# cbacary/MoDeGPT

Hardware: AMD Instinct MI355X
Metric: transformer layers compressed/sec (covariance+decomp+rebuild), Llama-3-8B @30% (higher is better)
Workload: dtype f64 from int8 MFMA digit planes, exact route: nine plane pairs + fp64 remainder sums, nothing truncated (error <= 5e-15 per call: fp64 rounding)

## Files before the change

modegpt_amd/csrc/common.hpp:

```cpp
#pragma once
#include <hip/hip_runtime.h>
#include <hip/hip_bf16.h>
#include <hip/hip_fp16.h>
#include <stdint.h>
#include <stdio.h>
#include <string.h>

#include "../../include/modegpt_hip.h"

namespace mdg {

typedef double d4 __attribute__((ext_vector_type(4)));
typedef double d2 __attribute__((ext_vector_type(2)));
typedef unsigned short bf16_t;
typedef unsigned short f16_t;

#ifdef MDG_EXPERIMENT
#define MDG_KNOB(name) (getenv(name) != nullptr)
#else
#define MDG_KNOB(name) false
#endif

void set_error(const char* fmt, ...);
enum { STATUS_NOT_PD = 1, STATUS_NO_CONVERGE = 2 };
int finish_flag(int* dflag, hipStream_t st, int kind, const char* what);

int release_i8_schedules();
int cov_accum_gated(const void* x, int dtype, int64_t n_tokens, int64_t n_feat, int64_t batch, int64_t ld, int relu, double* sigma,
                    int64_t ld_sigma, int64_t sigma_bs, void* ws, size_t ws_bytes, const int* gate, int gate_mask, int gate_want,
                    void* stream);
#define MDG_CHECK_ARG(cond, ...)            \
  do {                                      \
    if (!(cond)) {                          \
      mdg::set_error(__VA_ARGS__);          \
      return MDG_ERR_BAD_ARG;               \
    }                                       \
  } while (0)
#define MDG_HIP(call)                                                        \
  do {                                                                       \
    hipError_t e_ = (call);                                                  \
    if (e_ != hipSuccess) {                                                  \
      mdg::set_error("%s failed: %s (%s:%d)", #call, hipGetErrorString(e_),  \
                     __FILE__, __LINE__);                                    \
      return MDG_ERR_HIP;                                                    \
    }                                                                        \
  } while (0)
#define MDG_LAUNCH_CHECK() MDG_HIP(hipGetLastError())
#define MDG_CLEAR() (void)hipGetLastError()
#define MDG_TRY(call)              \
  do {                             \
    int s_ = (call);               \
    if (s_ != MDG_OK) return s_;   \
  } while (0)

__device__ __forceinline__ double bf16_to_f64(bf16_t b) {
  return (double)__uint_as_float(((unsigned)b) << 16);
}
__device__ __forceinline__ double f16_to_f64(f16_t h) {
  __half_raw r;
  r.x = h;
  return (double)__half2float(__half(r));
}
__device__ __forceinline__ bf16_t f64_to_bf16(double v) {
  float f = (float)v;
  unsigned u = __float_as_uint(f);
  if ((u & 0x7fffffffu) > 0x7f800000u) return (bf16_t)0x7fc0;
  u += 0x7fffu + ((u >> 16) & 1u);
  return (bf16_t)(u >> 16);
}

template <int DT> struct ElemOf;
template <> struct ElemOf<MDG_BF16> { typedef bf16_t type; };
template <> struct ElemOf<MDG_F16> { typedef f16_t type; };
template <> struct ElemOf<MDG_F32> { typedef float type; };
template <> struct ElemOf<MDG_F64> { typedef double type; };

template <int DT> __device__ __forceinline__ double load_f64(const void* p, int64_t i);
template <> __device__ __forceinline__ double load_f64<MDG_BF16>(const void* p, int64_t i) {
  return bf16_to_f64(((const bf16_t*)p)[i]);
}
template <> __device__ __forceinline__ double load_f64<MDG_F16>(const void* p, int64_t i) {
  return f16_to_f64(((const f16_t*)p)[i]);
}
template <> __device__ __forceinline__ double load_f64<MDG_F32>(const void* p, int64_t i) {
  return (double)((const float*)p)[i];
}
template <> __device__ __forceinline__ double load_f64<MDG_F64>(const void* p, int64_t i) {
  return ((const double*)p)[i];
}

static inline size_t dtype_size(int dt) {
  switch (dt) {
    case MDG_BF16: case MDG_F16: return 2;
    case MDG_F32: return 4;
    case MDG_F64: return 8;
  }
  return 0;
}

static inline int64_t ceil_div(int64_t a, int64_t b) { return (a + b - 1) / b; }
static inline size_t align_up(size_t a, size_t b) { return (a + b - 1) / b * b; }

constexpr int TILE = 128;
constexpr int WTILE = 64;
constexpr int BK = 16;
constexpr int PITCH = TILE + 2;
constexpr int PANEL = BK * PITCH;

struct Acc {
  d4 v[4][4];
};

__device__ __forceinline__ void acc_zero(Acc& a) {
#pragma unroll
  for (int i = 0; i < 4; i++)
#pragma unroll
    for (int j = 0; j < 4; j++) a.v[i][j] = (d4){0., 0., 0., 0.};
}

template <int K4_LO, int K4_HI>
__device__ __forceinline__ void mma_steps(const double* __restrict__ As, const double* __restrict__ Bs, int wr,
                                          int wc, int lane, Acc& acc) {
  const int m = lane & 15, kq = lane >> 4;
#pragma unroll
  for (int k4 = K4_LO; k4 < K4_HI; k4++) {
    const double* ap = As + (k4 * 4 + kq) * PITCH + wr * WTILE + 4 * m;
    const double* bp = Bs + (k4 * 4 + kq) * PITCH + wc * WTILE + 4 * m;
    d2 a01 = *(const d2*)ap, a23 = *(const d2*)(ap + 2);
    d2 b01 = *(const d2*)bp, b23 = *(const d2*)(bp + 2);
    double a[4] = {a01.x, a01.y, a23.x, a23.y};
    double b[4] = {b01.x, b01.y, b23.x, b23.y};
#pragma unroll
    for (int sa = 0; sa < 4; sa++)
#pragma unroll
      for (int sb = 0; sb < 4; sb++)
        acc.v[sa][sb] = __builtin_amdgcn_mfma_f64_16x16x4f64(a[sa], b[sb], acc.v[sa][sb], 0, 0, 0);
  }
}

__device__ __forceinline__ void mma_stage(const double* __restrict__ As, const double* __restrict__ Bs, int wr,
                                          int wc, int lane, Acc& acc) {
  mma_steps<0, BK / 4>(As, Bs, wr, wc, lane, acc);
}

__device__ __forceinline__ int acc_row(int wr, int lane, int sa, int reg) {
  return wr * WTILE + 4 * ((lane >> 4) + 4 * reg) + sa;
}
__device__ __forceinline__ int acc_col(int wc, int lane, int sb) { return wc * WTILE + 4 * (lane & 15) + sb; }

__device__ __forceinline__ void tri_decode(int t, int& bi, int& bj) {
  int i = (int)((sqrt(8.0 * (double)t + 1.0) - 1.0) * 0.5);
  while ((i + 1) * (i + 2) / 2 <= t) i++;
  while (i * (i + 1) / 2 > t) i--;
  bi = i;
  bj = t - i * (i + 1) / 2;
}

}
```

modegpt_amd/csrc/cov.hip:

```cpp
#include <stdlib.h>

#include <type_traits>

#include "common.hpp"

namespace mdg {

struct CovArgs {
  const void* x;
  int64_t ld, n_tokens;
  int n_feat, batch, tiles, ntri;
  double* sigma;
  int64_t ld_sigma, sigma_bs;
  int ksplit;
  int64_t tokens_per_split;
  double* partial;
  int vec_ok;
  const int* gate;
  int gate_mask, gate_want;
};

template <int DT> struct Stage {
  typedef typename ElemOf<DT>::type T;
  static constexpr int VEC = 16 / (int)sizeof(T);
  static constexpr int CPR = TILE / VEC;
  static constexpr int CPT = BK * CPR / 256;
  union Chunk {
    uint4 q;
    T e[VEC];
  };
  static constexpr int RG = VEC >= 8 ? 4 : (VEC == 4 ? 2 : 1);
  static constexpr int CG = 8 / RG;
  __device__ static __forceinline__ void chunk_rc(int c, int& row, int& col) {
    const int g = c >> 3, i = c & 7;
    row = (g % (BK / RG)) * RG + (i % RG);
    col = ((g / (BK / RG)) * CG + i / RG) * VEC;
  }
};

template <int DT, bool FAST, bool INB = false>
__device__ __forceinline__ void load_panel(const CovArgs& a, int64_t tok0, int64_t tok_end, int64_t col0,
                                           int col_lim, int tid, typename Stage<DT>::Chunk* regs) {
  typedef Stage<DT> S;
  typedef typename S::T T;
  const T* x = (const T*)a.x;
#pragma unroll
  for (int p = 0; p < S::CPT; p++) {
    int row, col;
    S::chunk_rc(tid + 256 * p, row, col);
    int64_t tok = tok0 + row;
    typename S::Chunk ch;
    ch.q = make_uint4(0, 0, 0, 0);
    if (FAST && INB) {
      ch.q = *(const uint4*)(x + tok * a.ld + col0 + col);
    } else if (FAST) {
      if (tok < tok_end) ch.q = *(const uint4*)(x + tok * a.ld + col0 + col);
    } else if (tok < tok_end) {
      const T* src = x + tok * a.ld + col0 + col;
      if (a.vec_ok && col + S::VEC <= col_lim) {
        ch.q = *(const uint4*)src;
      } else {
#pragma unroll
        for (int e = 0; e < S::VEC; e++)
          if (col + e < col_lim) ch.e[e] = src[e];
      }
    }
    regs[p] = ch;
  }
}

template <int DT, bool RELU>
__device__ __forceinline__ void store_panel(double* panel, int tid, const typename Stage<DT>::Chunk* regs) {
  typedef Stage<DT> S;
#pragma unroll
  for (int p = 0; p < S::CPT; p++) {
    int row, col;
    S::chunk_rc(tid + 256 * p, row, col);
    double* dst = panel + row * PITCH + col;
#pragma unroll
    for (int e = 0; e < S::VEC; e += 2) {
      double v0 = load_f64<DT>(regs[p].e, e), v1 = load_f64<DT>(regs[p].e, e + 1);
      if (RELU) {
        v0 = v0 > 0. ? v0 : 0.;
        v1 = v1 > 0. ? v1 : 0.;
      }
      *(d2*)(dst + e) = (d2){v0, v1};
    }
  }
}

template <int DT, bool RELU>
__device__ __forceinline__ void store_piece(double* panel, int tid, const typename Stage<DT>::Chunk* regs, int piece) {
  typedef Stage<DT> S;
  constexpr int PAIRS = S::CPT * S::VEC / 2;
  constexpr int PER = PAIRS / 4;
#pragma unroll
  for (int u = 0; u < PER; u++) {
    const int w = piece * PER + u;
    const int p = w / (S::VEC / 2), e = (w % (S::VEC / 2)) * 2;
    int row, col;
    S::chunk_rc(tid + 256 * p, row, col);
    double v0 = load_f64<DT>(regs[p].e, e), v1 = load_f64<DT>(regs[p].e, e + 1);
    if (RELU) {
      v0 = v0 > 0. ? v0 : 0.;
      v1 = v1 > 0. ? v1 : 0.;
    }
    *(d2*)(panel + row * PITCH + col + e) = (d2){v0, v1};
  }
}

template <int DT, bool RELU, bool DIAG>
__device__ __forceinline__ void mma_half_with_staging(const double* __restrict__ As, const double* __restrict__ Bs,
                                                      int wr, int wc, int lane, Acc& acc, bool stage_next,
                                                      double* nextA, double* nextB, int tid,
                                                      const typename Stage<DT>::Chunk* ra,
                                                      const typename Stage<DT>::Chunk* rb) {
  const int m = lane & 15, kq = lane >> 4;
  double a[2][4], b[2][4];
#pragma unroll
  for (int h = 0; h < 2; h++) {
    const int k4 = BK / 8 + h;
    const double* ap = As + (k4 * 4 + kq) * PITCH + wr * WTILE + 4 * m;
    const double* bp = Bs + (k4 * 4 + kq) * PITCH + wc * WTILE + 4 * m;
    d2 a01 = *(const d2*)ap, a23 = *(const d2*)(ap + 2);
    d2 b01 = *(const d2*)bp, b23 = *(const d2*)(bp + 2);
    a[h][0] = a01.x; a[h][1] = a01.y; a[h][2] = a23.x; a[h][3] = a23.y;
    b[h][0] = b01.x; b[h][1] = b01.y; b[h][2] = b23.x; b[h][3] = b23.y;
  }
#pragma unroll
  for (int h = 0; h < 2; h++)
#pragma unroll
    for (int sa = 0; sa < 4; sa++) {
#pragma unroll
      for (int sb = 0; sb < 4; sb++)
        acc.v[sa][sb] = __builtin_amdgcn_mfma_f64_16x16x4f64(a[h][sa], b[h][sb], acc.v[sa][sb], 0, 0, 0);
      if (stage_next) {
        const int piece = h * 4 + sa;
        if (piece < 4) store_piece<DT, RELU>(nextA, tid, ra, piece);
        else if (!DIAG) store_piece<DT, RELU>(nextB, tid, rb, piece - 4);
      }
      __builtin_amdgcn_sched_barrier(0);
    }
}

template <int DT, bool RELU, bool FAST, bool DIAG>
__device__ __forceinline__ void cov_tile(const CovArgs& a, double* lds, int b, int bi, int bj, int split, int slot) {
  typedef Stage<DT> S;
  const int tid = threadIdx.x, lane = tid & 63, wave = tid >> 6;
  const int wr = wave >> 1, wc = wave & 1;
  const int64_t tok_begin = (int64_t)split * a.tokens_per_split;
  int64_t tok_end = tok_begin + a.tokens_per_split;
  if (tok_end > a.n_tokens) tok_end = a.n_tokens;
  const int64_t colA = (int64_t)b * a.n_feat + (int64_t)bi * TILE;
  const int64_t colB = (int64_t)b * a.n_feat + (int64_t)bj * TILE;
  const int limA = min(TILE, a.n_feat - bi * TILE), limB = min(TILE, a.n_feat - bj * TILE);

  Acc acc;
  acc_zero(acc);
  typename S::Chunk ra1[S::CPT], rb1[S::CPT], ra2[S::CPT], rb2[S::CPT];
  const int64_t n_stage = tok_end > tok_begin ? (tok_end - tok_begin + BK - 1) / BK : 0;

  if (n_stage > 0) {
    load_panel<DT, FAST>(a, tok_begin, tok_end, colA, limA, tid, ra1);
    if (!DIAG) load_panel<DT, FAST>(a, tok_begin, tok_end, colB, limB, tid, rb1);
    store_panel<DT, RELU>(lds, tid, ra1);
    if (!DIAG) store_panel<DT, RELU>(lds + 2 * PANEL, tid, rb1);
    if (n_stage > 1) {
      load_panel<DT, FAST>(a, tok_begin + BK, tok_end, colA, limA, tid, ra1);
      if (!DIAG) load_panel<DT, FAST>(a, tok_begin + BK, tok_end, colB, limB, tid, rb1);
    }
  }
  __syncthreads();
  auto stage = [&](int64_t s, auto cur_c, auto steady_c, typename S::Chunk* st_a, typename S::Chunk* st_b,
                   typename S::Chunk* ld_a, typename S::Chunk* ld_b) {
    constexpr int CUR = decltype(cur_c)::value;
    constexpr bool STEADY = decltype(steady_c)::value;
    if (STEADY || s + 2 < n_stage) {
      const int64_t tk = tok_begin + (s + 2) * BK;
      load_panel<DT, FAST, STEADY>(a, tk, tok_end, colA, limA, tid, ld_a);
      if (!DIAG) load_panel<DT, FAST, STEADY>(a, tk, tok_end, colB, limB, tid, ld_b);
    }
    const double* As = lds + CUR * PANEL;
    const double* Bs = DIAG ? As : lds + (2 + CUR) * PANEL;
    mma_steps<0, BK / 8>(As, Bs, wr, wc, lane, acc);
    mma_half_with_staging<DT, RELU, DIAG>(As, Bs, wr, wc, lane, acc, STEADY || s + 1 < n_stage, lds + (CUR ^ 1) * PANEL,
                                          lds + (2 + (CUR ^ 1)) * PANEL, tid, st_a, st_b);
    __syncthreads();
  };
  using I0 = std::integral_constant<int, 0>;
  using I1 = std::integral_constant<int, 1>;
  int64_t s = 0;
  const int64_t n_full = (tok_end - tok_begin) / BK;
  for (; s + 3 < n_full; s += 2) {
    stage(s, I0{}, std::true_type{}, ra1, rb1, ra2, rb2);
    stage(s + 1, I1{}, std::true_type{}, ra2, rb2, ra1, rb1);
  }
  for (; s + 1 < n_stage; s += 2) {
    stage(s, I0{}, std::false_type{}, ra1, rb1, ra2, rb2);
    stage(s + 1, I1{}, std::false_type{}, ra2, rb2, ra1, rb1);
  }
  if (s < n_stage) stage(s, I0{}, std::false_type{}, ra1, rb1, ra2, rb2);

  if (a.ksplit == 1) {
    double* sg = a.sigma + (int64_t)b * a.sigma_bs;
#pragma unroll
    for (int sa = 0; sa < 4; sa++)
#pragma unroll
      for (int reg = 0; reg < 4; reg++) {
        int r = acc_row(wr, lane, sa, reg);
        int64_t gr = (int64_t)bi * TILE + r;
        if (gr >= a.n_feat) continue;
        int c0 = acc_col(wc, lane, 0);
        int64_t gc0 = (int64_t)bj * TILE + c0;
        double* row = sg + gr * a.ld_sigma + gc0;
#pragma unroll
        for (int sb = 0; sb < 4; sb++)
          if (gc0 + sb < a.n_feat) row[sb] += acc.v[sa][sb][reg];
      }
  } else {
    double* pt = a.partial + ((int64_t)split * (a.batch * a.ntri) + slot) * (TILE * TILE);
#pragma unroll
    for (int sa = 0; sa < 4; sa++)
#pragma unroll
      for (int reg = 0; reg < 4; reg++) {
        int r = acc_row(wr, lane, sa, reg);
        int c0 = acc_col(wc, lane, 0);
        d4 v = {acc.v[sa][0][reg], acc.v[sa][1][reg], acc.v[sa][2][reg], acc.v[sa][3][reg]};
        *(d4*)(pt + r * TILE + c0) = v;
      }
  }
}

template <int DT, bool RELU, bool FAST>
__global__ __launch_bounds__(256, 2) void cov_accum_kernel(CovArgs a) {
  __shared__ double lds[4 * PANEL];
  if (a.gate && (*a.gate & a.gate_mask) != a.gate_want) return;
  const int b = blockIdx.x / a.ntri, t = blockIdx.x % a.ntri;
  int bi, bj;
  tri_decode(t, bi, bj);
  if (bi == bj) cov_tile<DT, RELU, FAST, true>(a, lds, b, bi, bj, blockIdx.y, blockIdx.x);
  else cov_tile<DT, RELU, FAST, false>(a, lds, b, bi, bj, blockIdx.y, blockIdx.x);
}

constexpr int MULTI_MAX = 4;
struct CovMulti {
  int n;
  int unit_start[MULTI_MAX + 1];
  CovArgs p[MULTI_MAX];
};

template <int DT>
__global__ __launch_bounds__(256, 2) void cov_accum_multi_kernel(CovMulti m) {
  __shared__ double lds[4 * PANEL];
  int u = blockIdx.x, pi = 0;
  while (pi + 1 < m.n && u >= m.unit_start[pi + 1]) pi++;
  u -= m.unit_start[pi];
  const CovArgs& a = m.p[pi];
  const int tiles = a.batch * a.ntri;
  const int split = u / tiles, slot = u % tiles;
  const int b = slot / a.ntri, t = slot % a.ntri;
  int bi, bj;
  tri_decode(t, bi, bj);
  if (bi == bj) cov_tile<DT, false, true, true>(a, lds, b, bi, bj, split, slot);
  else cov_tile<DT, false, true, false>(a, lds, b, bi, bj, split, slot);
}

__global__ __launch_bounds__(256) void cov_reduce_kernel(CovArgs a) {
  if (a.gate && (*a.gate & a.gate_mask) != a.gate_want) return;
  const int b = blockIdx.x / a.ntri, t = blockIdx.x % a.ntri;
  int bi, bj;
  tri_decode(t, bi, bj);
  double* sg = a.sigma + (int64_t)b * a.sigma_bs;
  const int64_t tile_stride = (int64_t)gridDim.x * (TILE * TILE);
  const double* pt = a.partial + (int64_t)blockIdx.x * (TILE * TILE);
  const int e = blockIdx.y * 256 + threadIdx.x;
  const int r = e / TILE, c = e % TILE;
  const int64_t gr = (int64_t)bi * TILE + r, gc = (int64_t)bj * TILE + c;
  if (gr >= a.n_feat || gc >= a.n_feat) return;
  double s = 0.;
  for (int k = 0; k < a.ksplit; k++) s += pt[k * tile_stride + e];
  sg[gr * a.ld_sigma + gc] += s;
}

__global__ __launch_bounds__(256) void cov_finalize_kernel(double* sigma, int n, int64_t ld, int64_t bs, int tiles,
                                                           int ntri, double scale) {
  __shared__ double tl[32][33];
  const int b = blockIdx.x / ntri, t = blockIdx.x % ntri;
  int ti, tj;
  tri_decode(t, ti, tj);
  double* sg = sigma + (int64_t)b * bs;
  const int tx = threadIdx.x & 31, ty = threadIdx.x >> 5;
  for (int r = ty; r < 32; r += 8) {
    int gr = ti * 32 + r, gc = tj * 32 + tx;
    tl[r][tx] = (gr < n && gc < n) ? sg[(int64_t)gr * ld + gc] * scale : 0.;
  }
  __syncthreads();
  for (int r = ty; r < 32; r += 8) {
    int gr = ti * 32 + r, gc = tj * 32 + tx;
    if (gr < n && gc < n) {
      double v = (ti == tj && tx > r) ? tl[tx][r] : tl[r][tx];
      sg[(int64_t)gr * ld + gc] = v;
    }
    if (ti != tj) {
      int ur = tj * 32 + r, uc = ti * 32 + tx;
      if (ur < n && uc < n) sg[(int64_t)ur * ld + uc] = tl[tx][r];
    }
  }
}

template <int DT>
__global__ __launch_bounds__(256) void bi_partial_kernel(const void* xin, const void* xout, int64_t n_tokens,
                                                         int64_t d, int64_t ld, double* partial) {
  __shared__ double red[4];
  const int lane = threadIdx.x & 63, wave = threadIdx.x >> 6;
  double local = 0.;
  for (int64_t tok = (int64_t)blockIdx.x * 4 + wave; tok < n_tokens; tok += (int64_t)gridDim.x * 4) {
    double dot = 0., na = 0., nb = 0.;
    for (int64_t j = lane; j < d; j += 64) {
      double u = load_f64<DT>(xin, tok * ld + j), v = load_f64<DT>(xout, tok * ld + j);
      dot += u * v;
      na += u * u;
      nb += v * v;
    }
    for (int o = 32; o > 0; o >>= 1) {
      dot += __shfl_xor(dot, o);
      na += __shfl_xor(na, o);
      nb += __shfl_xor(nb, o);
    }
    const double eps = 1e-8;
    double den = fmax(sqrt(na), eps) * fmax(sqrt(nb), eps);
    local += 1.0 - dot / den;
  }
  if (lane == 0) red[wave] = local;
  __syncthreads();
  if (threadIdx.x == 0) partial[blockIdx.x] = red[0] + red[1] + red[2] + red[3];
}

__global__ void bi_final_kernel(const double* partial, int n, double* out) {
  if (threadIdx.x == 0 && blockIdx.x == 0) {
    double s = 0.;
    for (int i = 0; i < n; i++) s += partial[i];
    *out += s;
  }
}

static int cov_ksplit(int64_t n_tokens, int64_t n_feat, int64_t batch, int64_t* tokens_per_split) {
  const int64_t T = ceil_div(n_feat, TILE);
  const int64_t blocks = batch * T * (T + 1) / 2;
  const double slots = 512.0;
  const double us_per_token = 2.0 * TILE * TILE / (78.6e12 / slots) * 1e6;
  const double us_per_tile_rt = 2.0 * TILE * TILE * 8 / 4.0e12 * 1e6;
  int64_t max_split = n_tokens / (8 * BK);
  if (max_split < 1) max_split = 1;
  if (max_split > 256) max_split = 256;
  int64_t best = 1;
  double best_cost = 0.;
#ifdef MDG_EXPERIMENT
  if (const char* ev = getenv("MDG_COV_KSPLIT")) {
    const int64_t f = atoll(ev);
    if (f >= 1 && f <= max_split) {
      const int64_t tps = (int64_t)align_up((size_t)ceil_div(n_tokens, f), BK);
      *tokens_per_split = tps;
      return (int)ceil_div(n_tokens, tps);
    }
  }
#endif
  for (int64_t ks = 1; ks <= max_split; ks++) {
    const int64_t tps = (int64_t)align_up((size_t)ceil_div(n_tokens, ks), BK);
    const int64_t real = ceil_div(n_tokens, tps);
    if (real != ks) continue;
    double rounds = (double)ceil_div(blocks * ks, (int64_t)slots);
    double cost = rounds * (double)tps * us_per_token + (ks > 1 ? (double)(blocks * ks) * us_per_tile_rt + 3.0 : 0.);
    if (ks == 1 || cost < best_cost * (best == 1 ? 0.95 : 0.98)) {
      best = ks;
      best_cost = cost;
    }
  }
  int64_t tps = (int64_t)align_up((size_t)ceil_div(n_tokens > 0 ? n_tokens : 1, best), BK);
  *tokens_per_split = tps;
  return (int)ceil_div(n_tokens > 0 ? n_tokens : 1, tps);
}

template <int DT>
static void launch_cov(const CovArgs& a, int relu, bool fast, hipStream_t st) {
  dim3 grid(a.batch * a.ntri, a.ksplit);
  if (fast) {
    if (relu) hipLaunchKernelGGL((cov_accum_kernel<DT, true, true>), grid, dim3(256), 0, st, a);
    else hipLaunchKernelGGL((cov_accum_kernel<DT, false, true>), grid, dim3(256), 0, st, a);
  } else {
    if (relu) hipLaunchKernelGGL((cov_accum_kernel<DT, true, false>), grid, dim3(256), 0, st, a);
    else hipLaunchKernelGGL((cov_accum_kernel<DT, false, false>), grid, dim3(256), 0, st, a);
  }
}

}

using namespace mdg;

extern "C" size_t mdg_cov_accum_ws_bytes(int64_t n_tokens, int64_t n_feat, int64_t batch) {
  if (n_tokens <= 0 || n_feat <= 0 || batch <= 0) return 0;
  int64_t tps;
  int ks = cov_ksplit(n_tokens, n_feat, batch, &tps);
  if (ks == 1) return 0;
  int64_t T = ceil_div(n_feat, TILE);
  return (size_t)ks * batch * (T * (T + 1) / 2) * TILE * TILE * sizeof(double);
}

extern "C" int mdg_cov_accum(const void* x, int dtype, int64_t n_tokens, int64_t n_feat, int64_t batch,
                             int64_t ld, int relu, double* sigma, int64_t ld_sigma, int64_t sigma_bs, void* ws,
                             size_t ws_bytes, void* stream) {
  return mdg::cov_accum_gated(x, dtype, n_tokens, n_feat, batch, ld, relu, sigma, ld_sigma, sigma_bs, ws, ws_bytes, nullptr, 0, 0,
                              stream);
}

int mdg::cov_accum_gated(const void* x, int dtype, int64_t n_tokens, int64_t n_feat, int64_t batch, int64_t ld, int relu,
                         double* sigma, int64_t ld_sigma, int64_t sigma_bs, void* ws, size_t ws_bytes, const int* gate,
                         int gate_mask, int gate_want, void* stream) {
  MDG_CLEAR();
  MDG_CHECK_ARG(n_tokens >= 0 && n_feat > 0 && batch > 0, "mdg_cov_accum: bad sizes (tokens=%lld feat=%lld batch=%lld)",
                (long long)n_tokens, (long long)n_feat, (long long)batch);
  MDG_CHECK_ARG(dtype >= MDG_BF16 && dtype <= MDG_F64, "mdg_cov_accum: unknown dtype %d", dtype);
  MDG_CHECK_ARG(ld >= n_feat * batch, "mdg_cov_accum: ld %lld < batch*n_feat %lld", (long long)ld,
                (long long)(n_feat * batch));
  MDG_CHECK_ARG(ld_sigma >= n_feat, "mdg_cov_accum: ld_sigma %lld < n_feat", (long long)ld_sigma);
  MDG_CHECK_ARG(batch == 1 || sigma_bs >= n_feat * ld_sigma - (ld_sigma - n_feat),
                "mdg_cov_accum: sigma batch stride too small");
  MDG_CHECK_ARG(n_feat < (1 << 30) && batch * n_feat < (1ll << 31), "mdg_cov_accum: n_feat too large");
  if (n_tokens == 0) return MDG_OK;
  MDG_CHECK_ARG(x && sigma, "mdg_cov_accum: null pointer");
  hipStream_t st = (hipStream_t)stream;
  CovArgs a;
  a.x = x;
  a.ld = ld;
  a.n_tokens = n_tokens;
  a.n_feat = (int)n_feat;
  a.batch = (int)batch;
  a.tiles = (int)ceil_div(n_feat, TILE);
  a.ntri = a.tiles * (a.tiles + 1) / 2;
  a.sigma = sigma;
  a.ld_sigma = ld_sigma;
  a.sigma_bs = sigma_bs;
  a.ksplit = cov_ksplit(n_tokens, n_feat, batch, &a.tokens_per_split);
  a.partial = (double*)ws;
  a.gate = gate;
  a.gate_mask = gate_mask;
  a.gate_want = gate_want;
  size_t esz = dtype_size(dtype);
  a.vec_ok = ((uintptr_t)x % 16 == 0) && ((ld * esz) % 16 == 0) && ((n_feat * esz) % 16 == 0 || batch == 1);
  if (a.ksplit > 1) {
    size_t need = mdg_cov_accum_ws_bytes(n_tokens, n_feat, batch);
    MDG_CHECK_ARG(ws && ws_bytes >= need, "mdg_cov_accum: workspace %zu < required %zu", ws_bytes, need);
  }
  MDG_CHECK_ARG((int64_t)a.batch * a.ntri < (1ll << 31) && a.ksplit < 65536, "mdg_cov_accum: grid too large");
  const bool fast = a.vec_ok && (n_feat % TILE == 0);
  switch (dtype) {
    case MDG_BF16: launch_cov<MDG_BF16>(a, relu, fast, st); break;
    case MDG_F16: launch_cov<MDG_F16>(a, relu, fast, st); break;
    case MDG_F32: launch_cov<MDG_F32>(a, relu, fast, st); break;
    default: launch_cov<MDG_F64>(a, relu, fast, st); break;
  }
  MDG_LAUNCH_CHECK();
  if (a.ksplit > 1) {
    hipLaunchKernelGGL(cov_reduce_kernel, dim3(a.batch * a.ntri, TILE * TILE / 256), dim3(256), 0, st, a);
    MDG_LAUNCH_CHECK();
  }
  return MDG_OK;
}

static int multi_ksplit(int64_t n_tokens, int64_t* tokens_per_split) {
  int64_t ks = n_tokens / 4096;
  if (ks < 1) ks = 1;
  if (ks > 64) ks = 64;
  int64_t tps = (int64_t)align_up((size_t)ceil_div(n_tokens, ks), BK);
  *tokens_per_split = tps;
  return (int)ceil_div(n_tokens, tps);
}

static int multi_plan(int n, const mdg_cov_problem* pr, int dtype, CovMulti* m, size_t* ws_need) {
  MDG_CHECK_ARG(n >= 1 && n <= MULTI_MAX && pr, "mdg_cov_accum_multi: 1..%d problems", MULTI_MAX);
  MDG_CHECK_ARG(dtype >= MDG_BF16 && dtype <= MDG_F64, "mdg_cov_accum_multi: unknown dtype %d", dtype);
  const size_t esz = dtype_size(dtype);
  size_t off = 0;
  int64_t units = 0;
  m->n = n;
  for (int i = 0; i < n; i++) {
    const mdg_cov_problem& q = pr[i];
    MDG_CHECK_ARG(q.n_tokens > 0 && q.n_feat > 0 && q.batch > 0 && q.x && q.sigma, "mdg_cov_accum_multi: problem %d empty", i);
    MDG_CHECK_ARG(q.n_feat % TILE == 0 && q.ld >= q.n_feat * q.batch && q.ld_sigma >= q.n_feat,
                  "mdg_cov_accum_multi: problem %d needs n_feat %% 128 == 0 (got %lld) and consistent strides", i,
                  (long long)q.n_feat);
    MDG_CHECK_ARG((uintptr_t)q.x % 16 == 0 && (q.ld * esz) % 16 == 0,
                  "mdg_cov_accum_multi: problem %d is not 16-byte aligned (use mdg_cov_accum)", i);
    CovArgs& a = m->p[i];
    a.x = q.x; a.ld = q.ld; a.n_tokens = q.n_tokens; a.n_feat = (int)q.n_feat; a.batch = (int)q.batch;
    a.tiles = (int)(q.n_feat / TILE); a.ntri = a.tiles * (a.tiles + 1) / 2;
    a.sigma = q.sigma; a.ld_sigma = q.ld_sigma; a.sigma_bs = q.sigma_batch_stride; a.vec_ok = 1;
    a.gate = nullptr; a.gate_mask = a.gate_want = 0;
    const int64_t tiles = (int64_t)a.batch * a.ntri;
    if (i == 0 && tiles >= 768) { a.ksplit = 1; a.tokens_per_split = (int64_t)align_up((size_t)q.n_tokens, BK); }
    else a.ksplit = multi_ksplit(q.n_tokens, &a.tokens_per_split);
    a.partial = nullptr;
    m->unit_start[i] = (int)units;
    units += tiles * a.ksplit;
    MDG_CHECK_ARG(units < (1ll << 30), "mdg_cov_accum_multi: grid too large");
    if (a.ksplit > 1) {
      a.partial = (double*)off;
      off += (size_t)a.ksplit * tiles * TILE * TILE * sizeof(double);
    }
  }
  m->unit_start[n] = (int)units;
  *ws_need = off;
  return MDG_OK;
}

extern "C" size_t mdg_cov_accum_multi_ws_bytes(int n, const mdg_cov_problem* problems, int dtype) {
  CovMulti m;
  size_t need = 0;
  if (multi_plan(n, problems, dtype, &m, &need) != MDG_OK) return 0;
  return need;
}

extern "C" int mdg_cov_accum_multi(int n, const mdg_cov_problem* problems, int dtype, void* ws, size_t ws_bytes,
                                   void* stream) {
  MDG_CLEAR();
  CovMulti m;
  size_t need = 0;
  MDG_TRY(multi_plan(n, problems, dtype, &m, &need));
  MDG_CHECK_ARG(need == 0 || (ws && ws_bytes >= need), "mdg_cov_accum_multi: workspace %zu < required %zu", ws_bytes, need);
  for (int i = 0; i < n; i++)
    if (m.p[i].ksplit > 1) m.p[i].partial = (double*)((char*)ws + (size_t)m.p[i].partial);
  hipStream_t st = (hipStream_t)stream;
  dim3 grid((unsigned)m.unit_start[n]);
  switch (dtype) {
    case MDG_BF16: hipLaunchKernelGGL(cov_accum_multi_kernel<MDG_BF16>, grid, dim3(256), 0, st, m); break;
    case MDG_F16: hipLaunchKernelGGL(cov_accum_multi_kernel<MDG_F16>, grid, dim3(256), 0, st, m); break;
    case MDG_F32: hipLaunchKernelGGL(cov_accum_multi_kernel<MDG_F32>, grid, dim3(256), 0, st, m); break;
    default: hipLaunchKernelGGL(cov_accum_multi_kernel<MDG_F64>, grid, dim3(256), 0, st, m); break;
  }
  MDG_LAUNCH_CHECK();
  for (int i = 0; i < n; i++)
    if (m.p[i].ksplit > 1) {
      hipLaunchKernelGGL(cov_reduce_kernel, dim3(m.p[i].batch * m.p[i].ntri, TILE * TILE / 256), dim3(256), 0, st, m.p[i]);
      MDG_LAUNCH_CHECK();
    }
  return MDG_OK;
}

extern "C" int mdg_cov_finalize(double* sigma, int64_t n, int64_t batch, int64_t ld_sigma, int64_t sigma_bs,
                                double scale, void* stream) {
  MDG_CLEAR();
  MDG_CHECK_ARG(sigma && n > 0 && batch > 0 && ld_sigma >= n, "mdg_cov_finalize: bad arguments");
  int tiles = (int)ceil_div(n, 32);
  int64_t ntri = (int64_t)tiles * (tiles + 1) / 2;
  MDG_CHECK_ARG(batch * ntri < (1ll << 31), "mdg_cov_finalize: grid too large");
  hipLaunchKernelGGL(cov_finalize_kernel, dim3((unsigned)(batch * ntri)), dim3(256), 0, (hipStream_t)stream, sigma,
                     (int)n, ld_sigma, sigma_bs, tiles, (int)ntri, scale);
  MDG_LAUNCH_CHECK();
  return MDG_OK;
}

static const int BI_MAX_BLOCKS = 2048;
extern "C" size_t mdg_bi_ws_bytes(int64_t n_tokens) { return (size_t)BI_MAX_BLOCKS * sizeof(double); }

extern "C" int mdg_bi_accum(const void* x_in, const void* x_out, int dtype, int64_t n_tokens, int64_t d, int64_t ld,
                            double* out, void* ws, size_t ws_bytes, void* stream) {
  MDG_CLEAR();
  MDG_CHECK_ARG(x_in && x_out && out && n_tokens >= 0 && d > 0 && ld >= d, "mdg_bi_accum: bad arguments");
  MDG_CHECK_ARG(ws && ws_bytes >= mdg_bi_ws_bytes(n_tokens), "mdg_bi_accum: workspace too small");
  if (n_tokens == 0) return MDG_OK;
  int blocks = (int)(ceil_div(n_tokens, 4) < BI_MAX_BLOCKS ? ceil_div(n_tokens, 4) : BI_MAX_BLOCKS);
  hipStream_t st = (hipStream_t)stream;
  double* partial = (double*)ws;
  switch (dtype) {
    case MDG_BF16: hipLaunchKernelGGL(bi_partial_kernel<MDG_BF16>, dim3(blocks), dim3(256), 0, st, x_in, x_out, n_tokens, d, ld, partial); break;
    case MDG_F16: hipLaunchKernelGGL(bi_partial_kernel<MDG_F16>, dim3(blocks), dim3(256), 0, st, x_in, x_out, n_tokens, d, ld, partial); break;
    case MDG_F32: hipLaunchKernelGGL(bi_partial_kernel<MDG_F32>, dim3(blocks), dim3(256), 0, st, x_in, x_out, n_tokens, d, ld, partial); break;
    case MDG_F64: hipLaunchKernelGGL(bi_partial_kernel<MDG_F64>, dim3(blocks), dim3(256), 0, st, x_in, x_out, n_tokens, d, ld, partial); break;
    default: MDG_CHECK_ARG(false, "mdg_bi_accum: unknown dtype %d", dtype);
  }
  MDG_LAUNCH_CHECK();
  hipLaunchKernelGGL(bi_final_kernel, dim3(1), dim3(64), 0, st, partial, blocks, out);
  MDG_LAUNCH_CHECK();
  return MDG_OK;
}
```

modegpt_amd/csrc/cov_i8.hip:

```cpp
#include <algorithm>

#include "cov_i8.hpp"

namespace mdg {
namespace {

size_t layout(int count, const mdg_cov_problem* pr, void* ws, I8Call* out, size_t* fallback_off) {
  size_t off = SHARED_BYTES + PARTIAL_BYTES, fb = 0;
  char* const base = (char*)ws;
  if (out) {
    out->count = count;
    out->n_tokens = pr[0].n_tokens;
    out->nk = (int)ceil_div(pr[0].n_tokens, KS);
    out->shared = (SharedBlock*)base;
    out->partial = (double*)(base + SHARED_BYTES);
  }
  for (int i = 0; i < count; i++) {
    const int64_t cols = pr[i].n_feat * pr[i].batch, T = pr[i].n_tokens;
    const LoWsBytes lo = lo_ws_bytes(T, cols);
    I8Stat s;
    s.x = (const bf16_t*)pr[i].x; s.ld = pr[i].ld;
    s.sigma = pr[i].sigma; s.ld_sigma = pr[i].ld_sigma;
    s.n = (int)cols; s.block = pr[i].batch > 1 ? TI : 0;
    s.route_flag = out ? out->shared->route_flag + i : nullptr;
    auto take = [&](size_t bytes) { char* p = base ? base + off : nullptr; off += bytes; return p; };
    s.planes = (signed char*)take(align_up((size_t)NP * (size_t)cols * (size_t)ceil_div(T, KS) * KS, 256));
    s.emax = (int*)take(align_up(ints_bytes(cols), 256));
    s.vals = (double*)take(align_up(route_vals_bytes(cols), 256));
    s.route = (RouteOut*)take(align_up(sizeof(RouteOut), 256));
    s.colpart = (double*)take(align_up(column_partials_bytes(cols), 256));
    s.zmask = (unsigned char*)take(align_up((size_t)ceil_div(T, KS) * (size_t)(cols / 32), 256));
    s.lo_entries = (LoEntry*)take(lo.entries);
    s.lo_counts = (int*)take(align_up(lo.counts, 256));
    s.lo_xd = (bf16_t*)take(align_up(lo.xd, 256));
    s.lo_rentries = (LoEntry*)take(lo.rentries);
    s.lo_rtotals = (int*)take(align_up(lo.rtotals, 256));
    const RowsWsBytes rw = rows_ws_bytes(T);
    s.rowmask = (unsigned*)take(rw.mask);
    s.votes = (int*)take(rw.votes);
    s.rows_out = (RowsOut*)take(rw.out);
    if (out) out->stat[i] = s;
    fb = std::max(fb, mdg_cov_accum_ws_bytes(T, pr[i].n_feat, pr[i].batch));
  }
  if (fallback_off) *fallback_off = off;
  return off + fb + 256;
}

bool problems_ok(int count, const mdg_cov_problem* pr) {
  if (count < 1 || count > MAX_PROBLEMS || !pr) return false;
  for (int i = 0; i < count; i++) {
    if (pr[i].n_tokens != pr[0].n_tokens || pr[i].n_tokens < 0 || pr[i].n_tokens >= (1ll << 28) || pr[i].n_feat <= 0 || pr[i].batch < 1) return false;
    if (pr[i].batch == 1 ? pr[i].n_feat % TI != 0 : pr[i].n_feat != TI) return false;
    if (pr[i].n_feat * pr[i].batch >= (1 << 21)) return false;
    if (pr[i].ld < pr[i].n_feat * pr[i].batch || pr[i].ld_sigma < pr[i].n_feat) return false;
    if (pr[i].batch > 1 && (pr[i].ld_sigma != TI || pr[i].sigma_batch_stride != (int64_t)TI * TI)) return false;
  }
  return true;
}

}
}

using namespace mdg;

extern "C" size_t mdg_cov_accum_i8_multi_ws_bytes(int count, const mdg_cov_problem* problems) {
  if (!problems_ok(count, problems) || problems[0].n_tokens == 0) return 0;
  return layout(count, problems, nullptr, nullptr, nullptr);
}

extern "C" int mdg_cov_accum_i8_multi(int count, const mdg_cov_problem* problems, void* ws, size_t ws_bytes, double tolerance, int flags,
                                      int* used_i8, int* route_counts, void* ev_start, void* ev_stop, void* stream) {
  MDG_CLEAR();
  if (used_i8) *used_i8 = 0;
  MDG_CHECK_ARG(tolerance >= 1.0 && tolerance <= 1e6, "mdg_cov_accum_i8_multi: tolerance factor %g outside [1, 1e6] (1 = guaranteed <= 1.1e-11)",
                tolerance);
  MDG_CHECK_ARG((flags & ~(MDG_I8_NO_EXACT | MDG_I8_EXACT_ALWAYS | MDG_I8_F16 | MDG_I8_RELU | MDG_I8_ROWS)) == 0 &&
                    (flags & (MDG_I8_NO_EXACT | MDG_I8_EXACT_ALWAYS)) != (MDG_I8_NO_EXACT | MDG_I8_EXACT_ALWAYS),
                "mdg_cov_accum_i8_multi: bad flags 0x%x", flags);
  bool offer_exact = !(flags & MDG_I8_NO_EXACT);
  const bool exact_always = (flags & MDG_I8_EXACT_ALWAYS) != 0;
  for (int i = 0; i < count; i++)
    if ((uint64_t)problems[i].n_tokens * (uint64_t)problems[i].ld * 2ull >= (1ull << 32)) offer_exact = false;
  MDG_CHECK_ARG(problems_ok(count, problems),
                "mdg_cov_accum_i8_multi: 1..%d statistics of the same token count; full ones need n_feat %% 128 == 0, per-head ones "
                "head_dim 128 with contiguous [heads][128][128] sigma; leading dimensions at least the widths (use mdg_cov_accum)",
                MAX_PROBLEMS);
  if (problems[0].n_tokens == 0) return MDG_OK;
  for (int i = 0; i < count; i++) MDG_CHECK_ARG(problems[i].x && problems[i].sigma, "mdg_cov_accum_i8_multi: null pointer");
  I8Call c;
  size_t fb_off = 0;
  const size_t need = layout(count, problems, ws, &c, &fb_off);
  MDG_CHECK_ARG(ws && ws_bytes >= need, "mdg_cov_accum_i8_multi: workspace %zu < required %zu", ws_bytes, need);
  c.route_counts = route_counts;
  c.st = (hipStream_t)stream;
  c.f16 = (flags & MDG_I8_F16) != 0;
  c.relu = (flags & MDG_I8_RELU) != 0;
  c.rows = (flags & MDG_I8_ROWS) != 0;
  MDG_HIP(hipMemsetAsync(c.shared, 0, SHARED_BYTES, c.st));
  if (c.rows) MDG_HIP(hipMemsetAsync(&c.shared->rows_flag, 1, 1, c.st));
  for (int i = 0; i < count; i++) {
    MDG_TRY(enqueue_split(c, i));
    MDG_TRY(enqueue_route(c, i, tolerance));
  }
  if (offer_exact) MDG_TRY(enqueue_lo_lists(c, exact_always));
  MDG_TRY(enqueue_products(c, offer_exact, ev_start, ev_stop));
  if (offer_exact) MDG_TRY(enqueue_lo_products(c, exact_always));
  for (int i = 0; i < count; i++) MDG_TRY(enqueue_columns(c, i));
  if (c.rows)
    for (int i = 0; i < count; i++) MDG_TRY(enqueue_rows_product(c, i));
  for (int i = 0; i < count; i++) {
    const mdg_cov_problem& q = problems[i];
    MDG_TRY(cov_accum_gated(q.x, c.f16 ? MDG_F16 : MDG_BF16, c.n_tokens, q.n_feat, q.batch, q.ld, c.relu ? 1 : 0, q.sigma, q.ld_sigma, q.sigma_batch_stride, (char*)ws + fb_off,
                            ws_bytes - fb_off, c.stat[i].route_flag, 2, 2, stream));
  }
  MDG_TRY(report_product_diagnostics(c));
  if (used_i8) {
    int pf[MAX_PROBLEMS] = {};
    MDG_HIP(hipMemcpyAsync(pf, c.shared->route_flag, sizeof(pf), hipMemcpyDeviceToHost, c.st));
    MDG_HIP(hipStreamSynchronize(c.st));
    int live = 0, six = 0;
    for (int i = 0; i < count; i++)
      if (!(pf[i] & 2)) {
        live++;
        six |= pf[i] & 1;
      }
    *used_i8 = live ? (six ? 6 : 5) : 0;
  }
  return MDG_OK;
}

static mdg_cov_problem single_problem(const void* x, int64_t n_tokens, int64_t n_feat, int64_t ld, double* sigma, int64_t ld_sigma) {
  mdg_cov_problem q;
  q.x = x; q.n_tokens = n_tokens; q.n_feat = n_feat; q.batch = 1; q.ld = ld;
  q.sigma = sigma; q.ld_sigma = ld_sigma; q.sigma_batch_stride = 0;
  return q;
}

extern "C" size_t mdg_cov_accum_i8_ws_bytes(int64_t n_tokens, int64_t n_feat) {
  if (n_tokens <= 0 || n_feat <= 0) return 0;
  const mdg_cov_problem q = single_problem(nullptr, n_tokens, n_feat, n_feat, nullptr, n_feat);
  return mdg_cov_accum_i8_multi_ws_bytes(1, &q);
}

extern "C" int mdg_cov_accum_i8(const void* x, int64_t n_tokens, int64_t n_feat, int64_t ld, double* sigma, int64_t ld_sigma,
                                void* ws, size_t ws_bytes, double tolerance, int flags, int* used_i8, int* route_counts, void* ev_start,
                                void* ev_stop, void* stream) {
  MDG_CLEAR();
  if (used_i8) *used_i8 = 0;
  MDG_CHECK_ARG(n_tokens >= 0 && n_feat > 0, "mdg_cov_accum_i8: bad sizes (tokens=%lld feat=%lld)", (long long)n_tokens,
                (long long)n_feat);
  MDG_CHECK_ARG(n_feat % TI == 0, "mdg_cov_accum_i8: n_feat=%lld must be a multiple of %d (use mdg_cov_accum)",
                (long long)n_feat, TI);
  const mdg_cov_problem q = single_problem(x, n_tokens, n_feat, ld, sigma, ld_sigma);
  return mdg_cov_accum_i8_multi(1, &q, ws, ws_bytes, tolerance, flags, used_i8, route_counts, ev_start, ev_stop, stream);
}

extern "C" int mdg_cov_accum_i8_route(int count, const mdg_cov_problem* problems, int stat, const void* ws, int* planes, int* n_columns,
                                      int* columns, double* bound, int* exact, void* stream) {
  MDG_CLEAR();
  MDG_CHECK_ARG(problems_ok(count, problems) && stat >= 0 && stat < count && ws, "mdg_cov_accum_i8_route: bad arguments");
  I8Call c;
  layout(count, problems, const_cast<void*>(ws), &c, nullptr);
  RouteOut r;
  SharedBlock shared;
  hipStream_t st = (hipStream_t)stream;
  MDG_HIP(hipMemcpyAsync(&r, c.stat[stat].route, sizeof(r), hipMemcpyDeviceToHost, st));
  MDG_HIP(hipMemcpyAsync(&shared, c.shared, sizeof(shared), hipMemcpyDeviceToHost, st));
  MDG_HIP(hipStreamSynchronize(st));
  const bool was_exact = r.planes != 0 && shared.exact_ran == 1 && shared.exact_overflow == 0;
  int rows_left = 0;
  if (shared.rows_flag && r.planes != 0) {
    RowsOut ro;
    MDG_HIP(hipMemcpyAsync(&ro, c.stat[stat].rows_out, sizeof(ro), hipMemcpyDeviceToHost, st));
    MDG_HIP(hipStreamSynchronize(st));
    rows_left = ro.n_rows;
  }
  if (exact) *exact = was_exact ? shared.exact_mode : 0;
  if (planes) *planes = r.planes;
  if (n_columns) *n_columns = r.n_out;
  if (columns)
    for (int i = 0; i < MDG_I8_MAX_COLUMNS; i++) columns[i] = i < r.n_out ? r.out[i] : -1;
  if (bound) {
    bound[0] = was_exact ? r.rho + MDG_I8_EXACT_ROUNDING : r.sq;
    bound[1] = was_exact ? 0.0 : r.x;
    if (rows_left) bound[0] += (double)(rows_left + 1) * 0x1p-53;
  }
  return MDG_OK;
}

static int read_rows(const I8Call& c, int stat, RowsOut* out, hipStream_t st) {
  SharedBlock shared;
  MDG_HIP(hipMemcpyAsync(&shared, c.shared, sizeof(shared), hipMemcpyDeviceToHost, st));
  MDG_HIP(hipStreamSynchronize(st));
  out->n_rows = out->n_dominant = 0;
  if (!shared.rows_flag || (shared.route_flag[stat] & 2)) return MDG_OK;
  MDG_HIP(hipMemcpyAsync(out, c.stat[stat].rows_out, sizeof(*out), hipMemcpyDeviceToHost, st));
  MDG_HIP(hipStreamSynchronize(st));
  return MDG_OK;
}

extern "C" int mdg_cov_accum_i8_rows(int count, const mdg_cov_problem* problems, int stat, const void* ws, int* n_rows, int* rows,
                                     void* stream) {
  MDG_CLEAR();
  MDG_CHECK_ARG(problems_ok(count, problems) && stat >= 0 && stat < count && ws, "mdg_cov_accum_i8_rows: bad arguments");
  I8Call c;
  layout(count, problems, const_cast<void*>(ws), &c, nullptr);
  RowsOut r;
  MDG_TRY(read_rows(c, stat, &r, (hipStream_t)stream));
  if (n_rows) *n_rows = r.n_rows;
  if (rows)
    for (int i = 0; i < MDG_I8_MAX_ROWS; i++) rows[i] = i < r.n_rows ? r.rows[i] : -1;
  return MDG_OK;
}

extern "C" int mdg_cov_accum_i8_stats(const void* ws, int64_t n_tokens, int64_t n_feat, unsigned long long* executed_mfma,
                                      void* stream) {
  MDG_CLEAR();
  (void)n_tokens;
  (void)n_feat;
  MDG_CHECK_ARG(ws && executed_mfma, "mdg_cov_accum_i8_stats: bad arguments");
  const SharedBlock* shared = (const SharedBlock*)ws;
  hipStream_t st = (hipStream_t)stream;
  MDG_HIP(hipMemcpyAsync(executed_mfma, &shared->mfma_count, sizeof(unsigned long long), hipMemcpyDeviceToHost, st));
  MDG_HIP(hipStreamSynchronize(st));
  return MDG_OK;
}
```

modegpt_amd/csrc/cov_i8.hpp:

```cpp
#pragma once
#include <cstddef>

#include "common.hpp"

namespace mdg {

typedef int i32x4 __attribute__((ext_vector_type(4)));

constexpr int NP = 6;
constexpr int TI = 128;
constexpr int KS = 32;
constexpr int FLUSH_STEPS = 2047;
constexpr int FLUSH_STEPS_F16 = 2047;
static_assert(FLUSH_STEPS <= FLUSH_STEPS_F16, "the product kernels' fold interval must hold for fp16 elements too");
constexpr int TOP_SHIFT = 8 * NP - 10;
constexpr int TOP_SHIFT_F16 = 8 * NP - 13;

struct Bf16Elem {
  static constexpr int TOP = TOP_SHIFT, SIG_BITS = 8;
  static __device__ __forceinline__ void parts(unsigned b, int& sig, int& ee) {
    const int e = (b >> 7) & 0xFF, m = b & 0x7F;
    sig = e ? (128 | m) : m;
    ee = e ? e : 1;
    if (b & 0x8000) sig = -sig;
  }
  static __device__ __forceinline__ int ee_if_nonzero(unsigned b) {
    const int e = (b >> 7) & 0xFF;
    return (b & 0x7FFF) ? (e ? e : 1) : 0;
  }
  static __device__ __forceinline__ bool is_nan(unsigned b) { return (b & 0x7FFFu) > 0x7F80u; }
  static __device__ __forceinline__ double to_f64(unsigned b) { return (double)__uint_as_float(b << 16); }
  static __device__ __forceinline__ double lo_f64(unsigned w) { return (double)__uint_as_float(w << 16); }
  static __device__ __forceinline__ double hi_f64(unsigned w) { return (double)__uint_as_float(w & 0xFFFF0000u); }
  static __device__ __forceinline__ unsigned from_f64(double v) { return __float_as_uint((float)v) >> 16; }
  static __device__ __forceinline__ unsigned deep_limit(int E) { return (unsigned)max(E - 14, 1) << 7; }
};
struct F16Elem {
  static constexpr int TOP = TOP_SHIFT_F16, SIG_BITS = 11;
  static __device__ __forceinline__ void parts(unsigned b, int& sig, int& ee) {
    const int e = (b >> 10) & 0x1F, m = b & 0x3FF;
    sig = e ? (1024 | m) : m;
    ee = e == 31 ? 255 : (e ? e : 1) + 112;
    if (b & 0x8000) sig = -sig;
  }
  static __device__ __forceinline__ int ee_if_nonzero(unsigned b) {
    const int e = (b >> 10) & 0x1F;
    return (b & 0x7FFF) ? (e == 31 ? 255 : (e ? e : 1) + 112) : 0;
  }
  static __device__ __forceinline__ bool is_nan(unsigned b) { return (b & 0x7FFFu) > 0x7C00u; }
  static __device__ __forceinline__ double to_f64(unsigned b) { return f16_to_f64((f16_t)b); }
  static __device__ __forceinline__ double lo_f64(unsigned w) { return f16_to_f64((f16_t)(w & 0xFFFFu)); }
  static __device__ __forceinline__ double hi_f64(unsigned w) { return f16_to_f64((f16_t)(w >> 16)); }
  static __device__ __forceinline__ unsigned from_f64(double v) { return __half_as_ushort(__float2half((float)v)); }
  static __device__ __forceinline__ unsigned deep_limit(int E) { return (unsigned)max(E - 123, 1) << 10; }
};
template <class EL, bool RELU>
__device__ __forceinline__ unsigned relu_bits(unsigned b) {
  return (RELU && (b & 0x8000u) && !EL::is_nan(b)) ? 0u : b;
}
template <class EL, bool RELU>
__device__ __forceinline__ unsigned relu_pair(unsigned w) {
  if (!RELU) return w;
  return relu_bits<EL, true>(w & 0xFFFFu) | (relu_bits<EL, true>(w >> 16) << 16);
}
#define MDG_I8_DISPATCH(c, KERNEL, ...)                                                   \
  do {                                                                                    \
    if ((c).f16) {                                                                        \
      if ((c).relu) hipLaunchKernelGGL((KERNEL<F16Elem, true>), __VA_ARGS__);             \
      else hipLaunchKernelGGL((KERNEL<F16Elem, false>), __VA_ARGS__);                     \
    } else {                                                                              \
      if ((c).relu) hipLaunchKernelGGL((KERNEL<Bf16Elem, true>), __VA_ARGS__);            \
      else hipLaunchKernelGGL((KERNEL<Bf16Elem, false>), __VA_ARGS__);                    \
    }                                                                                     \
  } while (0)

#define MDG_I8_DISPATCH_ROWS(c, KERNEL, ...)                                              \
  do {                                                                                    \
    if ((c).rows) {                                                                       \
      if ((c).f16) {                                                                      \
        if ((c).relu) hipLaunchKernelGGL((KERNEL<F16Elem, true, true>), __VA_ARGS__);     \
        else hipLaunchKernelGGL((KERNEL<F16Elem, false, true>), __VA_ARGS__);             \
      } else {                                                                            \
        if ((c).relu) hipLaunchKernelGGL((KERNEL<Bf16Elem, true, true>), __VA_ARGS__);    \
        else hipLaunchKernelGGL((KERNEL<Bf16Elem, false, true>), __VA_ARGS__);            \
      }                                                                                   \
    } else if ((c).f16) {                                                                 \
      if ((c).relu) hipLaunchKernelGGL((KERNEL<F16Elem, true, false>), __VA_ARGS__);      \
      else hipLaunchKernelGGL((KERNEL<F16Elem, false, false>), __VA_ARGS__);              \
    } else {                                                                              \
      if ((c).relu) hipLaunchKernelGGL((KERNEL<Bf16Elem, true, false>), __VA_ARGS__);     \
      else hipLaunchKernelGGL((KERNEL<Bf16Elem, false, false>), __VA_ARGS__);             \
    }                                                                                     \
  } while (0)
template <bool ROWS>
__device__ __forceinline__ bool row_left(const unsigned* rowmask, int64_t t) {
  return ROWS && ((rowmask[t >> 5] >> (t & 31)) & 1u);
}

constexpr int NSTAT = 8;
constexpr int STAT_D0D1 = 6, STAT_COUNTS = 7;
constexpr int EMAX_COLUMN_OUT = 0x100;

constexpr int ALWAYS_WRITTEN_PLANES = 4;

constexpr int MAX_PROBLEMS = 4;
constexpr int ROUTE_JMAX = MDG_I8_MAX_COLUMNS;
constexpr int TAIL_MAX_PIECES = 1024;
constexpr size_t PARTIAL_BYTES = (size_t)TAIL_MAX_PIECES * TI * 128 * sizeof(double);

struct RouteOut {
  int planes;
  int n_out;
  int out[ROUTE_JMAX];
  double sq, x;
  double rho;
};
constexpr int ROWS_MAX = MDG_I8_MAX_ROWS;
struct RowsOut {
  int n_rows;
  int n_dominant;
  int rows[ROWS_MAX];
};
struct RouteScratch {
  int ticket, forced;
};

constexpr size_t SHARED_BYTES = 256;
struct SharedBlock {
  int reserved[2];
  unsigned long long mfma_count;
  int xcd_queue[8];
  int route_flag[MAX_PROBLEMS];
  int exact_overflow, exact_ran, exact_mode;
  int rows_flag;
};
static_assert(offsetof(SharedBlock, mfma_count) == 8 && offsetof(SharedBlock, xcd_queue) == 16 && offsetof(SharedBlock, route_flag) == 48 &&
                  offsetof(SharedBlock, exact_overflow) == 64 && offsetof(SharedBlock, exact_ran) == 68 &&
                  offsetof(SharedBlock, exact_mode) == 72 && sizeof(SharedBlock) <= SHARED_BYTES,
              "the shared block's layout is fixed");

struct LoEntry;
struct I8Stat {
  const bf16_t* x;
  int64_t ld;
  double* sigma;
  int64_t ld_sigma;
  int n, block;
  int* route_flag;
  signed char* planes;
  int* emax;
  unsigned char* zmask;
  double* vals;
  RouteOut* route;
  double* colpart;
  LoEntry *lo_entries, *lo_rentries;
  int *lo_counts, *lo_rtotals;
  bf16_t* lo_xd;
  unsigned* rowmask;
  int* votes;
  RowsOut* rows_out;
  bool vec() const { return (uintptr_t)x % 16 == 0 && ld % 8 == 0; }
  unsigned long long* stats() const { return (unsigned long long*)(emax + (n + 1) / 2 * 2); }
};
struct I8Call {
  int count, nk;
  int64_t n_tokens;
  I8Stat stat[MAX_PROBLEMS];
  bool f16, relu;
  bool rows;
  SharedBlock* shared;
  double* partial;
  int* route_counts;
  hipStream_t st;
};

inline size_t ints_bytes(int64_t n) { return (size_t)((n + 1) / 2 * 2) * sizeof(int) + (size_t)(NSTAT * n) * sizeof(unsigned long long) + sizeof(RouteScratch); }

#pragma GCC visibility push(hidden)
int enqueue_split(const I8Call& c, int i);
int enqueue_colmax(const I8Call& c, int i, bool masked);
struct RowsWsBytes { size_t mask, votes, out; };
RowsWsBytes rows_ws_bytes(int64_t n_tokens);
int enqueue_row_selection(const I8Call& c, int i);
int enqueue_rows_product(const I8Call& c, int i);
size_t route_vals_bytes(int64_t n);
size_t column_partials_bytes(int64_t n);
int enqueue_route(const I8Call& c, int i, double tolerance);
int enqueue_columns(const I8Call& c, int i);
struct LoWsBytes { size_t entries, counts, xd, rentries, rtotals; };
LoWsBytes lo_ws_bytes(int64_t n_tokens, int64_t n);
int enqueue_lo_lists(const I8Call& c, bool always);
int enqueue_lo_products(const I8Call& c, bool always);
int enqueue_products(const I8Call& c, bool offer_exact, void* ev_start, void* ev_stop);
int report_product_diagnostics(const I8Call& c);
#pragma GCC visibility pop

}
```

modegpt_amd/csrc/cov_i8_route.hip:

```cpp
#include <algorithm>

#include "cov_i8.hpp"

namespace mdg {
namespace {

constexpr double TAU_SQ = 1e-12, TAU_X_MIN = 1e-12, TAU_X_MAX = 1e-11, TAU_X_TOKENS = 1024.0;
__host__ __device__ inline double tau_x_of(int64_t tokens) {
  return fmin(TAU_X_MAX, fmax(TAU_X_MIN, TAU_X_MIN * ((double)tokens / TAU_X_TOKENS)));
}
constexpr int NVAL = 7;
constexpr int ROUTE_THREADS = 512;

__device__ __forceinline__ void route_terms(const double (&A)[NVAL], int P, double& sq, double& x) {
  sq = 2.0 * A[6] + A[6] * A[6];
  x = 0.0;
#pragma unroll
  for (int s = 0; s < NP; s++)
#pragma unroll
    for (int t = 0; t < NP; t++)
      if (s + t >= P) {
        if (s == t) sq += A[s] * A[t];
        else x += A[s] * A[t];
      }
}
__device__ __forceinline__ double route_violation(const double (&A)[NVAL], int P, double tau_x) {
  double sq, x;
  route_terms(A, P, sq, x);
  return fmax(sq / TAU_SQ, x / tau_x);
}

struct Top2 { double m1; int a1; double m2; };
__device__ __forceinline__ void top2_merge(Top2& a, const Top2& b) {
  if (b.m1 > a.m1 || (b.m1 == a.m1 && b.a1 < a.a1)) {
    a.m2 = fmax(a.m1, b.m2);
    a.m1 = b.m1;
    a.a1 = b.a1;
  } else {
    a.m2 = fmax(a.m2, b.m1);
  }
}

struct RoutePartial {
  Top2 top[NVAL];
  unsigned long long cls[NVAL][64];
  unsigned min_nnz;
};

__global__ __launch_bounds__(ROUTE_THREADS) void i8_route_kernel(const unsigned long long* __restrict__ stats, int* emax, int n, int64_t n_tokens,
                                                                 double* __restrict__ vals, RoutePartial* partial, RouteScratch* scratch,
                                                                 int* flag, RouteOut* out, int* route_counts, double tolerance) {
  __shared__ unsigned long long group_max[NVAL][64];
  __shared__ Top2 wave_top[ROUTE_THREADS / 64][NVAL];
  __shared__ Top2 top[NVAL];
  __shared__ double floor_of[NVAL];
  __shared__ int decision;
  __shared__ int forced_total, my_ticket;
  __shared__ unsigned min_nnz;
  __shared__ double tau_x_shared;
  const int tid = threadIdx.x, lane = tid & 63, wave = tid >> 6;
  for (int i = tid; i < NVAL * 64; i += ROUTE_THREADS) (&group_max[0][0])[i] = 0ull;
  if (tid == 0) min_nnz = 0xffffffffu;
  __syncthreads();
  auto reduce_top = [&](Top2 (&t)[NVAL]) {
#pragma unroll
    for (int i = 0; i < NVAL; i++) {
#pragma unroll
      for (int off = 32; off >= 1; off >>= 1) {
        Top2 o;
        o.m1 = __shfl_xor(t[i].m1, off);
        o.a1 = __shfl_xor(t[i].a1, off);
        o.m2 = __shfl_xor(t[i].m2, off);
        top2_merge(t[i], o);
      }
      if (lane == 0) wave_top[wave][i] = t[i];
    }
    __syncthreads();
    if (tid < NVAL) {
      Top2 r = wave_top[0][tid];
      for (int w = 1; w < ROUTE_THREADS / 64; w++) top2_merge(r, wave_top[w][tid]);
      top[tid] = r;
    }
    __syncthreads();
  };
  Top2 t[NVAL];
#pragma unroll
  for (int i = 0; i < NVAL; i++) t[i] = Top2{-1.0, 0x7fffffff, -1.0};
  {
    const int j = blockIdx.x * ROUTE_THREADS + tid;
    bool nonfinite = false;
    if (j < n) {
      double q[NSTAT];
#pragma unroll
      for (int i = 0; i < NSTAT - 1; i++) q[i] = i == STAT_D0D1 ? (double)(long long)stats[(int64_t)i * n + j] : (double)stats[(int64_t)i * n + j];
      const unsigned long long counts = stats[(int64_t)STAT_COUNTS * n + j];
      const int ex = emax[j];
      const double nnz = (double)(unsigned)counts, rounded = (double)(unsigned)(counts >> 32);
      const double hi2 = 65536.0 * q[0] + 512.0 * q[STAT_D0D1] + q[1];
      const double norm = (sqrt(fmax(hi2, 0.0)) - 0.5 * sqrt(nnz)) * 4294967296.0;
      const double inv = nnz > 0 ? (norm > 0 ? 1.0 / norm : 1e300) : 0.0;
      double a[NVAL];
#pragma unroll
      for (int s2 = 0; s2 < NP; s2++) a[s2] = q[s2] > 0 ? sqrt(q[s2]) * ldexp(1.0, 8 * (NP - 1 - s2)) * inv : 0.0;
      a[6] = rounded > 0 ? 0.5 * sqrt(rounded) * inv : 0.0;
      nonfinite = (ex & 255) == 255;
      if ((unsigned)counts) atomicMin(&min_nnz, (unsigned)counts);
#pragma unroll
      for (int i = 0; i < NVAL; i++) {
        vals[(int64_t)i * n + j] = a[i];
        if (!nonfinite) t[i] = Top2{a[i], j, -1.0};
      }
      if (nonfinite) emax[j] = ex | EMAX_COLUMN_OUT;
    }
#pragma unroll
    for (int i = 0; i < NVAL; i++)
      if (t[i].m1 > 0.0) atomicMax(&group_max[i][lane], (unsigned long long)__double_as_longlong(t[i].m1));
    const unsigned long long nf = __ballot(nonfinite);
    if (lane == 0 && nf) atomicAdd(&scratch->forced, __popcll(nf));
  }
  reduce_top(t);
  RoutePartial& mine = partial[blockIdx.x];
  if (tid < NVAL) mine.top[tid] = top[tid];
  if (tid == 0) mine.min_nnz = min_nnz;
  for (int i = tid; i < NVAL * 64; i += ROUTE_THREADS) (&mine.cls[0][0])[i] = (&group_max[0][0])[i];
  __threadfence();
  __syncthreads();
  if (tid == 0) my_ticket = atomicAdd(&scratch->ticket, 1);
  __syncthreads();
  if (my_ticket != (int)gridDim.x - 1) return;
  __threadfence();
  const unsigned nwg = gridDim.x;
  if (tid < NVAL) {
    Top2 r = partial[0].top[tid];
    unsigned w = 1;
    for (; w + 4 <= nwg; w += 4) {
      const Top2 b0 = partial[w].top[tid], b1 = partial[w + 1].top[tid], b2 = partial[w + 2].top[tid], b3 = partial[w + 3].top[tid];
      top2_merge(r, b0); top2_merge(r, b1); top2_merge(r, b2); top2_merge(r, b3);
    }
    for (; w < nwg; w++) top2_merge(r, partial[w].top[tid]);
    r.m1 = fmax(r.m1, 0.0);
    r.m2 = fmax(r.m2, 0.0);
    top[tid] = r;
  }
  for (int i = tid; i < NVAL * 64; i += ROUTE_THREADS) {
    unsigned long long m = 0ull;
    unsigned w = 0;
    for (; w + 4 <= nwg; w += 4) {
      const unsigned long long v0 = (&partial[w].cls[0][0])[i], v1 = (&partial[w + 1].cls[0][0])[i], v2 = (&partial[w + 2].cls[0][0])[i],
                               v3 = (&partial[w + 3].cls[0][0])[i];
      m = max(max(m, v0), max(max(v1, v2), v3));
    }
    for (; w < nwg; w++) m = max(m, (&partial[w].cls[0][0])[i]);
    (&group_max[0][0])[i] = m;
  }
  if (tid == 0) {
    forced_total = scratch->forced;
    unsigned m = 0xffffffffu;
    unsigned w = 0;
    for (; w + 4 <= nwg; w += 4) {
      const unsigned v0 = partial[w].min_nnz, v1 = partial[w + 1].min_nnz, v2 = partial[w + 2].min_nnz, v3 = partial[w + 3].min_nnz;
      m = min(min(m, v0), min(min(v1, v2), v3));
    }
    for (; w < nwg; w++) m = min(m, partial[w].min_nnz);
    tau_x_shared = tau_x_of(min(n_tokens, (int64_t)m));
  }
  __syncthreads();
  const double tau_x = tau_x_shared;
  int n_out = 0;
  if (forced_total > ROUTE_JMAX) {
    if (tid == 0) {
      out->planes = 0; out->n_out = 0; out->sq = out->x = out->rho = 0.0;
      atomicOr(flag, 2);
    }
    for (int j = tid; j < n; j += ROUTE_THREADS) emax[j] &= 255;
    return;
  }
  if (forced_total) {
    if (tid == 0)
      for (int j = 0; j < n; j++)
        if (emax[j] & EMAX_COLUMN_OUT) out->out[n_out++] = j;
    __syncthreads();
  }
  const int n_forced = forced_total;
  if (wave == 0) {
    const int want = ROUTE_JMAX - n_forced;
#pragma unroll 1
    for (int i = 0; i < NVAL; i++) {
      const unsigned long long mine = group_max[i][lane];
      int rank = 0;
      for (int k = 0; k < 64; k++) {
        const unsigned long long o = group_max[i][k];
        rank += (o > mine || (o == mine && k < lane));
      }
      if (rank == want) floor_of[i] = __longlong_as_double((long long)mine);
    }
  }
  __syncthreads();
  double fl[NVAL];
#pragma unroll
  for (int i = 0; i < NVAL; i++) fl[i] = floor_of[i];
  bool top_valid = true;
  for (int P = 5; P <= 6; P++) {
    if (n > 64 && route_violation(fl, P, tau_x) > tolerance) continue;
    n_out = n_forced;
    for (;;) {
      if (!top_valid) {
        top_valid = true;
#pragma unroll
        for (int i = 0; i < NVAL; i++) t[i] = Top2{-1.0, 0x7fffffff, -1.0};
        constexpr int PASS1_COLS = 4;
        for (int j0 = tid; j0 < n; j0 += ROUTE_THREADS * PASS1_COLS) {
          double v[PASS1_COLS][NVAL];
          int ex[PASS1_COLS];
#pragma unroll
          for (int c = 0; c < PASS1_COLS; c++) {
            const int j = j0 + c * ROUTE_THREADS;
            ex[c] = j < n ? emax[j] : EMAX_COLUMN_OUT;
#pragma unroll
            for (int i = 0; i < NVAL; i++) v[c][i] = j < n ? vals[(int64_t)i * n + j] : 0.0;
          }
#pragma unroll
          for (int c = 0; c < PASS1_COLS; c++)
            if (!(ex[c] & EMAX_COLUMN_OUT)) {
#pragma unroll
              for (int i = 0; i < NVAL; i++) top2_merge(t[i], Top2{v[c][i], j0 + c * ROUTE_THREADS, -1.0});
            }
        }
        reduce_top(t);
      }
      if (tid == 0) {
        double A[NVAL];
#pragma unroll
        for (int i = 0; i < NVAL; i++) {
          top[i].m1 = fmax(top[i].m1, 0.0);
          top[i].m2 = fmax(top[i].m2, 0.0);
          A[i] = top[i].m1;
        }
        decision = -1;
        if (route_violation(A, P, tau_x) <= tolerance) {
          out->planes = P;
          out->n_out = n_out;
          route_terms(A, P, out->sq, out->x);
          out->rho = 2.0 * A[6] + A[6] * A[6];
          if (P == 6) atomicOr(flag, 1);
          if (route_counts && n_out) atomicAdd(route_counts + 3, n_out);
          decision = 0;
        } else if (n_out == ROUTE_JMAX) {
          decision = 1;
        } else {
          int best = -1;
          double best_v = 1e308;
          for (int qi = 0; qi < NVAL; qi++) {
            const int c = top[qi].a1;
            if (c == 0x7fffffff) continue;
            double A2[NVAL];
#pragma unroll
            for (int i = 0; i < NVAL; i++) A2[i] = top[i].a1 == c ? top[i].m2 : top[i].m1;
            const double v = route_violation(A2, P, tau_x);
            if (v < best_v) { best_v = v; best = c; }
          }
          if (best < 0) decision = 1;
          else {
            emax[best] |= EMAX_COLUMN_OUT;
            out->out[n_out] = best;
          }
        }
      }
      __syncthreads();
      const int dec = decision;
      __syncthreads();
      if (dec == 0) return;
      if (dec == 1) break;
      n_out++;
      top_valid = false;
    }
    if (n_out > n_forced) {
      for (int j = tid; j < n; j += ROUTE_THREADS)
        if ((emax[j] & EMAX_COLUMN_OUT) && (emax[j] & 255) != 255) emax[j] &= 255;
      top_valid = false;
      __syncthreads();
    }
  }
  if (tid == 0) {
    out->planes = 0; out->n_out = 0; out->sq = out->x = out->rho = 0.0;
    atomicOr(flag, 2);
  }
  for (int j = tid; j < n; j += ROUTE_THREADS) emax[j] &= 255;
}

__global__ __launch_bounds__(256) void i8_clear_columns_kernel(const RouteOut* route, const int* flag, const int* emax, signed char* planes,
                                                               unsigned char* zmask, int n, int nk) {
  if ((*flag & 2) || (int)blockIdx.x >= route->n_out) return;
  const int j = route->out[blockIdx.x];
  const int64_t groups = n / 32;
  const int G = j >> 5, lane = threadIdx.x & 63, row = lane & 31;
  const bool row_out = (emax[G * 32 + row] & EMAX_COLUMN_OUT) != 0;
  for (int kt = blockIdx.y * 4 + (threadIdx.x >> 6); kt < nk; kt += gridDim.y * 4) {
    const unsigned old_mask = zmask[(int64_t)kt * groups + G];
    unsigned new_mask = 0;
#pragma unroll
    for (int s = 0; s < NP; s++) {
      if (s >= ALWAYS_WRITTEN_PLANES && (old_mask >> s) == 0) continue;
      i32x4* p = (i32x4*)(planes + ((s * groups + G) * (int64_t)nk + kt) * 1024) + lane;
      i32x4 v = *p;
      if (row_out) {
        v = (i32x4)0;
        *p = v;
      }
      if (__ballot((v[0] | v[1] | v[2] | v[3]) != 0)) new_mask |= 1u << s;
    }
    if (lane == 0) zmask[(int64_t)kt * groups + G] = (unsigned char)new_mask;
  }
}

constexpr int COLK_GROUP = 8, COLK_CHUNKS = 64, COLK_WG_COLS = 512, COLK_STAGE = 64, COLK_BATCH = 8;
struct ColArgs {
  const bf16_t* x;
  int64_t ld, T;
  int n, vec;
  const RouteOut* route;
  const int* flag;
  double* part;
  const unsigned* rowmask;
};

template <class EL, bool RELU, bool ROWS>
__global__ __launch_bounds__(64) void i8_columns_kernel(ColArgs a) {
  const int pass = blockIdx.z;
  const int n_out = a.route->n_out;
  if ((*a.flag & 2) || pass * COLK_GROUP >= n_out) return;
  const int nj = min(COLK_GROUP, n_out - pass * COLK_GROUP);
  __shared__ __attribute__((aligned(16))) double xj[COLK_STAGE][COLK_GROUP];
  const int lane = threadIdx.x;
  const int my_k = lane % COLK_GROUP;
  const int my_col = my_k < nj ? a.route->out[pass * COLK_GROUP + my_k] : -1;
  const int c0 = blockIdx.x * COLK_WG_COLS + lane * 8;
  const bool active = c0 < a.n;
  const int64_t chunk_len = (a.T + COLK_CHUNKS - 1) / COLK_CHUNKS;
  const int64_t t0 = blockIdx.y * chunk_len, t1 = min(a.T, t0 + chunk_len);
  const unsigned short* xs = (const unsigned short*)a.x;
  auto fetch_group = [&](int64_t t, unsigned short (&g)[COLK_STAGE / 8]) {
#pragma unroll
    for (int i = 0; i < COLK_STAGE / 8; i++) {
      const int64_t tok = t + lane / COLK_GROUP + 8 * i;
      g[i] = (my_col >= 0 && tok < t1 && !row_left<ROWS>(a.rowmask, tok)) ? (unsigned short)relu_bits<EL, RELU>(xs[tok * a.ld + my_col])
                                                                         : (unsigned short)0;
    }
  };
  double acc[COLK_GROUP][8] = {};
  unsigned short g[COLK_STAGE / 8];
  if (t0 < t1) fetch_group(t0, g);
  for (int64_t t = t0; t < t1; t += COLK_STAGE) {
    __syncthreads();
#pragma unroll
    for (int i = 0; i < COLK_STAGE / 8; i++) xj[lane / COLK_GROUP + 8 * i][my_k] = EL::to_f64(g[i]);
    __syncthreads();
    if (t + COLK_STAGE < t1) fetch_group(t + COLK_STAGE, g);
    if (!active) continue;
    const int steps = (int)min((int64_t)COLK_STAGE, t1 - t);
    for (int tb = 0; tb < steps; tb += COLK_BATCH) {
      unsigned w[COLK_BATCH][4];
#pragma unroll
      for (int i = 0; i < COLK_BATCH; i++) {
        const bool in_chunk = t + tb + i < t1;
        const int64_t tok = in_chunk ? t + tb + i : t1 - 1;
        const bool live = in_chunk && !row_left<ROWS>(a.rowmask, tok);
        if (a.vec) {
          const i32x4 v = *(const i32x4*)(xs + tok * a.ld + c0);
          w[i][0] = v[0]; w[i][1] = v[1]; w[i][2] = v[2]; w[i][3] = v[3];
        } else {
#pragma unroll
          for (int h = 0; h < 4; h++) w[i][h] = xs[tok * a.ld + c0 + 2 * h] | ((unsigned)xs[tok * a.ld + c0 + 2 * h + 1] << 16);
        }
        if (!live) w[i][0] = w[i][1] = w[i][2] = w[i][3] = 0u;
      }
#pragma unroll
      for (int i = 0; i < COLK_BATCH; i++) {
        double xc[8];
#pragma unroll
        for (int h = 0; h < 4; h++) {
          const unsigned wr = relu_pair<EL, RELU>(w[i][h]);
          xc[2 * h] = EL::to_f64(wr & 0xFFFFu);
          xc[2 * h + 1] = EL::to_f64(wr >> 16);
        }
#pragma unroll
        for (int k = 0; k < COLK_GROUP; k++) {
          const double xk = xj[tb + i][k];
#pragma unroll
          for (int c = 0; c < 8; c++) acc[k][c] += xk * xc[c];
        }
      }
    }
  }
  if (!active) return;
#pragma unroll
  for (int k = 0; k < COLK_GROUP; k++)
    if (k < nj) {
      double* o = a.part + ((int64_t)(pass * COLK_GROUP + k) * COLK_CHUNKS + blockIdx.y) * a.n + c0;
#pragma unroll
      for (int c = 0; c < 8; c++) o[c] = acc[k][c];
    }
}

__global__ __launch_bounds__(256) void i8_columns_reduce_kernel(ColArgs a, const int* emax, double* sigma, int64_t ld_sigma, int block) {
  const int k = blockIdx.y;
  if ((*a.flag & 2) || k >= a.route->n_out) return;
  const int c = blockIdx.x * 256 + threadIdx.x;
  if (c >= a.n) return;
  const int j = a.route->out[k];
  if (block && c / block != j / block) return;
  if ((emax[c] & EMAX_COLUMN_OUT) && c < j) return;
  double v = 0.0;
  for (int q = 0; q < COLK_CHUNKS; q++) v += a.part[((int64_t)k * COLK_CHUNKS + q) * a.n + c];
  const int row = max(c, j), col = min(c, j);
  sigma[(int64_t)row * ld_sigma + col - (block ? row / block * block : 0)] += v;
}

}

size_t route_vals_bytes(int64_t n) { return (size_t)(NVAL * n) * sizeof(double) + (size_t)ceil_div(n, (int64_t)ROUTE_THREADS) * sizeof(RoutePartial); }
size_t column_partials_bytes(int64_t n) { return (size_t)ROUTE_JMAX * COLK_CHUNKS * (size_t)n * sizeof(double); }

int enqueue_route(const I8Call& c, int i, double tolerance) {
  const I8Stat& s = c.stat[i];
  const int n = s.n;
  RoutePartial* partial = (RoutePartial*)(s.vals + (size_t)NVAL * n);
  RouteScratch* scratch = (RouteScratch*)(s.stats() + (size_t)NSTAT * n);
  hipLaunchKernelGGL(i8_route_kernel, dim3((unsigned)ceil_div(n, ROUTE_THREADS)), dim3(ROUTE_THREADS), 0, c.st, s.stats(), s.emax, n,
                     c.n_tokens, s.vals, partial, scratch, s.route_flag, s.route, c.route_counts, tolerance);
  hipLaunchKernelGGL(i8_clear_columns_kernel, dim3(ROUTE_JMAX, (unsigned)std::min(64, (c.nk + 3) / 4)), dim3(256), 0, c.st,
                     (const RouteOut*)s.route, (const int*)s.route_flag, (const int*)s.emax, s.planes, s.zmask, n, c.nk);
  MDG_LAUNCH_CHECK();
  return MDG_OK;
}

int enqueue_columns(const I8Call& c, int i) {
  const I8Stat& s = c.stat[i];
  ColArgs a;
  a.x = s.x; a.ld = s.ld; a.T = c.n_tokens; a.n = s.n;
  a.vec = s.vec();
  a.route = s.route;
  a.flag = s.route_flag;
  a.part = s.colpart;
  a.rowmask = s.rowmask;
  MDG_I8_DISPATCH_ROWS(c, i8_columns_kernel, dim3((unsigned)ceil_div(s.n, COLK_WG_COLS), COLK_CHUNKS, ROUTE_JMAX / COLK_GROUP), dim3(64), 0, c.st, a);
  hipLaunchKernelGGL(i8_columns_reduce_kernel, dim3((unsigned)ceil_div(s.n, 256), ROUTE_JMAX), dim3(256), 0, c.st, a, (const int*)s.emax, s.sigma,
                     s.ld_sigma, s.block);
  MDG_LAUNCH_CHECK();
  return MDG_OK;
}

}
```

modegpt_amd/csrc/cov_i8_rows.hip:

```cpp
#include <algorithm>

#include "cov_i8.hpp"

namespace mdg {
namespace {

constexpr int ROW_WINDOW = 4;
constexpr int ROW_SHARE = 8;
constexpr int ROW_MINORITY = 8;
constexpr int VOTE_SPAN = 1024;
constexpr int VOTE_TOKENS = 128;
constexpr int SELECT_THREADS = 1024;

template <class EL, bool RELU>
__global__ __launch_bounds__(256) void i8_row_votes_kernel(const bf16_t* x, int64_t ld, int64_t T, int n, int vec, const int* emax,
                                                           int* votes) {
  __shared__ __attribute__((aligned(16))) int thr[VOTE_SPAN];
  const int c_begin = blockIdx.y * VOTE_SPAN;
  const int span = min(VOTE_SPAN, n - c_begin);
  for (int i = threadIdx.x; i < span; i += 256) thr[i] = max((emax[c_begin + i] & 255) - ROW_WINDOW, 1);
  __syncthreads();
  const int cg = threadIdx.x & 15, tl = threadIdx.x >> 4;
  const int64_t slab0 = (int64_t)blockIdx.x * VOTE_TOKENS, t1 = min(T, slab0 + VOTE_TOKENS);
  for (int64_t tb = slab0; tb < t1; tb += 16) {
    const int64_t t = tb + tl;
    const bool live = t < t1;
    int cnt = 0;
    if (live) {
      const bf16_t* row = x + t * ld + c_begin;
#pragma unroll
      for (int cb = 0; cb < VOTE_SPAN / 128; cb++) {
        const int jl = cb * 128 + cg * 8;
        if (jl >= span) break;
        unsigned w[4];
        if (vec) {
          const i32x4 v = *(const i32x4*)(row + jl);
          w[0] = v[0]; w[1] = v[1]; w[2] = v[2]; w[3] = v[3];
        } else {
#pragma unroll
          for (int h = 0; h < 4; h++) w[h] = row[jl + 2 * h] | ((unsigned)row[jl + 2 * h + 1] << 16);
        }
        const i32x4 h0 = *(const i32x4*)(thr + jl), h1 = *(const i32x4*)(thr + jl + 4);
        const int th[8] = {h0[0], h0[1], h0[2], h0[3], h1[0], h1[1], h1[2], h1[3]};
#pragma unroll
        for (int q = 0; q < 4; q++) {
          const unsigned wr = relu_pair<EL, RELU>(w[q]);
          cnt += (EL::ee_if_nonzero(wr & 0xFFFFu) >= th[2 * q]) + (EL::ee_if_nonzero(wr >> 16) >= th[2 * q + 1]);
        }
      }
    }
#pragma unroll
    for (int off = 1; off < 16; off <<= 1) cnt += __shfl_xor(cnt, off);
    if (live && cg == 0 && cnt) atomicAdd(votes + t, cnt);
  }
}

__global__ __launch_bounds__(SELECT_THREADS) void i8_row_select_kernel(const int* votes, int64_t T, int n, unsigned* rowmask, RowsOut* out,
                                                                       int* emax) {
  __shared__ int cnt[SELECT_THREADS];
  const int tid = threadIdx.x;
  const int64_t chunk = (T + SELECT_THREADS - 1) / SELECT_THREADS;
  const int64_t a = min(T, tid * chunk), b = min(T, a + chunk);
  const int need = n / ROW_SHARE;
  int mine = 0;
  for (int64_t t = a; t < b; t++) mine += votes[t] >= need;
  cnt[tid] = mine;
  __syncthreads();
  for (int off = 1; off < SELECT_THREADS; off <<= 1) {
    const int v = tid >= off ? cnt[tid - off] : 0;
    __syncthreads();
    cnt[tid] += v;
    __syncthreads();
  }
  const int n_dom = cnt[SELECT_THREADS - 1];
  const bool leave = n_dom >= 1 && n_dom <= ROWS_MAX && (int64_t)n_dom * ROW_MINORITY <= T;
  if (tid == 0) {
    out->n_dominant = n_dom;
    out->n_rows = leave ? n_dom : 0;
  }
  if (!leave) return;
  int k = cnt[tid] - mine;
  if (mine)
    for (int64_t t = a; t < b; t++)
      if (votes[t] >= need) {
        out->rows[k++] = (int)t;
        atomicOr(rowmask + (t >> 5), 1u << (t & 31));
      }
  for (int j = tid; j < n; j += SELECT_THREADS) emax[j] = 0;
}

struct RowArgs {
  const bf16_t* x;
  int64_t ld;
  int block;
  const RowsOut* rows;
  const int* flag;
  double* sigma;
  int64_t ld_sigma;
  int* route_counts;
};

template <class EL, bool RELU>
__global__ __launch_bounds__(256) void i8_rows_product_kernel(RowArgs a) {
  __shared__ __attribute__((aligned(16))) double lds[2 * PANEL];
  __shared__ int tok[ROWS_MAX];
  const int nr = a.rows->n_rows;
  if (nr == 0 || (*a.flag & 2)) return;
  int bi, bj;
  if (a.block) bi = bj = blockIdx.x;
  else tri_decode(blockIdx.x, bi, bj);
  const int tid = threadIdx.x, lane = tid & 63, wave = tid >> 6;
  const int wr = wave >> 1, wc = wave & 1;
  if (tid < ROWS_MAX) tok[tid] = tid < nr ? a.rows->rows[tid] : -1;
  if (blockIdx.x == 0 && tid == 0 && a.route_counts) atomicAdd(a.route_counts + 5, nr);
  __syncthreads();
  const bool diag = bi == bj;
  double* const As = lds;
  double* const Bs = diag ? lds : lds + PANEL;
  const unsigned short* xs = (const unsigned short*)a.x;
  Acc acc;
  acc_zero(acc);
  for (int k0 = 0; k0 < nr; k0 += BK) {
    if (k0) __syncthreads();
#pragma unroll
    for (int i = 0; i < BK / 2; i++) {
      const int k = (tid >> 7) + 2 * i, f = tid & 127;
      const int t = tok[k0 + k];
      double va = 0., vb = 0.;
      if (t >= 0) {
        const unsigned short* row = xs + (int64_t)t * a.ld;
        va = EL::to_f64(relu_bits<EL, RELU>(row[bi * TILE + f]));
        if (!diag) vb = EL::to_f64(relu_bits<EL, RELU>(row[bj * TILE + f]));
      }
      As[k * PITCH + f] = va;
      if (!diag) Bs[k * PITCH + f] = vb;
    }
    __syncthreads();
    mma_stage(As, Bs, wr, wc, lane, acc);
  }
#pragma unroll
  for (int sa = 0; sa < 4; sa++)
#pragma unroll
    for (int reg = 0; reg < 4; reg++) {
      const int gr = bi * TILE + acc_row(wr, lane, sa, reg);
      const int gc0 = bj * TILE + acc_col(wc, lane, 0);
      double* row = a.sigma + (int64_t)gr * a.ld_sigma + gc0 - (a.block ? gr / a.block * a.block : 0);
#pragma unroll
      for (int sb = 0; sb < 4; sb++)
        if (gc0 + sb <= gr) row[sb] += acc.v[sa][sb][reg];
    }
}

}

RowsWsBytes rows_ws_bytes(int64_t n_tokens) {
  RowsWsBytes b;
  b.mask = align_up((size_t)ceil_div(n_tokens, (int64_t)32) * sizeof(unsigned), 256);
  b.votes = align_up((size_t)n_tokens * sizeof(int), 256);
  b.out = align_up(sizeof(RowsOut), 256);
  return b;
}

int enqueue_row_selection(const I8Call& c, int i) {
  const I8Stat& s = c.stat[i];
  const RowsWsBytes b = rows_ws_bytes(c.n_tokens);
  MDG_HIP(hipMemsetAsync(s.rowmask, 0, b.mask + b.votes + b.out, c.st));
  MDG_I8_DISPATCH(c, i8_row_votes_kernel, dim3((unsigned)ceil_div(c.n_tokens, (int64_t)VOTE_TOKENS), (unsigned)ceil_div(s.n, VOTE_SPAN)),
                  dim3(256), 0, c.st, s.x, s.ld, c.n_tokens, s.n, (int)s.vec(), (const int*)s.emax, s.votes);
  hipLaunchKernelGGL(i8_row_select_kernel, dim3(1), dim3(SELECT_THREADS), 0, c.st, (const int*)s.votes, c.n_tokens, s.n, s.rowmask,
                     s.rows_out, s.emax);
  MDG_LAUNCH_CHECK();
  return MDG_OK;
}

int enqueue_rows_product(const I8Call& c, int i) {
  const I8Stat& s = c.stat[i];
  RowArgs a;
  a.x = s.x; a.ld = s.ld; a.block = s.block;
  a.rows = s.rows_out;
  a.flag = s.route_flag;
  a.sigma = s.sigma; a.ld_sigma = s.ld_sigma;
  a.route_counts = c.route_counts;
  const int64_t nb = s.n / TILE;
  MDG_I8_DISPATCH(c, i8_rows_product_kernel, dim3((unsigned)(s.block ? nb : nb * (nb + 1) / 2)), dim3(256), 0, c.st, a);
  MDG_LAUNCH_CHECK();
  return MDG_OK;
}

}
```

modegpt_amd/csrc/cov_i8_split.hip:

```cpp
#include <algorithm>

#include "cov_i8.hpp"

namespace mdg {
namespace {

template <class EL>
__device__ __forceinline__ long long fixed_point(int sig, int sh, bool& rounded) {
  rounded = sh > EL::TOP;
  if (!rounded) return (long long)sig << (EL::TOP - sh);
  const int dn = sh - EL::TOP;
  const int mag = dn > EL::SIG_BITS + 1 ? 0 : ((sig < 0 ? -sig : sig) + (1 << (dn - 1))) >> dn;
  return sig < 0 ? -mag : mag;
}

template <class EL, bool RELU, bool ROWS>
__global__ __launch_bounds__(256) void i8_colmax_kernel(const bf16_t* x, int64_t ld, int64_t T, int n, int64_t rows_per_block,
                                                        int* emax, const unsigned* rowmask, const RowsOut* rows_out) {
  if (ROWS && rows_out->n_rows == 0) return;
  const int j = blockIdx.x * 64 + (threadIdx.x & 63);
  const int64_t t0 = (int64_t)blockIdx.y * rows_per_block + (threadIdx.x >> 6);
  const int64_t t1 = min(T, (int64_t)(blockIdx.y + 1) * rows_per_block);
  int best = 1;
  if (j < n)
    for (int64_t t = t0; t < t1; t += 4) {
      int sig, ee;
      EL::parts(relu_bits<EL, RELU>(x[t * ld + j]), sig, ee);
      if (sig != 0 && !row_left<ROWS>(rowmask, t)) best = max(best, ee);
    }
  if (j < n) atomicMax(emax + j, best);
}

__device__ __forceinline__ unsigned write_piece_mask(const unsigned (&any)[NP], unsigned char* zmask, int64_t index) {
  unsigned byte = 0;
#pragma unroll
  for (int s = 0; s < NP; s++) {
    const unsigned long long b = __ballot(any[s] != 0);
    const unsigned half = (threadIdx.x & 32) ? (unsigned)(b >> 32) : (unsigned)b;
    byte |= (half != 0) << s;
  }
  if ((threadIdx.x & 31) == 0) zmask[index] = (unsigned char)byte;
  return byte;
}

constexpr int SPLIT_STEPS = 64;
template <class EL, bool RELU, bool ROWS>
__global__ __launch_bounds__(256) void i8_split_kernel(const bf16_t* x, int64_t ld, int64_t T, int n, int nk, const int* emax,
                                                       signed char* planes, unsigned long long* stats, unsigned char* zmask,
                                                       const unsigned* rowmask) {
  __shared__ unsigned long long st_lds[NSTAT][32];
  const int r = threadIdx.x & 31;
  const int G = blockIdx.x;
  const int j = G * 32 + r;
  const int E = emax[j];
  const int64_t groups = n / 32;
  for (int i = threadIdx.x; i < NSTAT * 32; i += 256) (&st_lds[0][0])[i] = 0;
  __syncthreads();
  long long q[NSTAT] = {};
  for (int kq = 0; kq < SPLIT_STEPS; kq += 8) {
    const int kt = blockIdx.y * SPLIT_STEPS + kq + (threadIdx.x >> 5);
    if (kt >= nk) break;
    unsigned any[NP] = {};
#pragma unroll
    for (int h = 0; h < 2; h++) {
      unsigned dig[NP][4] = {};
#pragma unroll
      for (int qq = 0; qq < 16; qq++) {
        const int64_t t = (int64_t)kt * KS + h * 16 + qq;
        int sig = 0, ee = 1;
        if (t < T && !row_left<ROWS>(rowmask, t)) EL::parts(relu_bits<EL, RELU>(x[t * ld + j]), sig, ee);
        bool rounded;
        long long N = fixed_point<EL>(sig, E - ee, rounded);
        q[STAT_COUNTS] += (long long)(sig != 0) + ((long long)(sig != 0 && rounded) << 32);
        int d[NP];
#pragma unroll
        for (int s = NP - 1; s >= 1; s--) {
          d[s] = (int)((N + 128) & 255) - 128;
          dig[s][qq >> 2] |= (unsigned)(d[s] & 255) << (8 * (qq & 3));
          N = (N - d[s]) >> 8;
        }
        d[0] = (int)N;
        dig[0][qq >> 2] |= (unsigned)(d[0] & 255) << (8 * (qq & 3));
#pragma unroll
        for (int s = 0; s < NP; s++) q[s] += d[s] * d[s];
        q[STAT_D0D1] += d[0] * d[1];
      }
#pragma unroll
      for (int s = 0; s < NP; s++) {
        signed char* piece = planes + ((s * groups + G) * (int64_t)nk + kt) * 1024;
        *(i32x4*)(piece + h * 512 + r * 16) = (i32x4){(int)dig[s][0], (int)dig[s][1], (int)dig[s][2], (int)dig[s][3]};
        any[s] |= dig[s][0] | dig[s][1] | dig[s][2] | dig[s][3];
      }
    }
    write_piece_mask(any, zmask, (int64_t)kt * groups + G);
  }
#pragma unroll
  for (int i = 0; i < NSTAT; i++)
    if (q[i]) atomicAdd(&st_lds[i][r], (unsigned long long)q[i]);
  __syncthreads();
  for (int i = threadIdx.x; i < NSTAT * 32; i += 256)
    if (st_lds[i >> 5][i & 31]) atomicAdd(stats + (int64_t)(i >> 5) * n + G * 32 + (i & 31), st_lds[i >> 5][i & 31]);
}

#ifndef MDG_COLMAX_WGS
#define MDG_COLMAX_WGS 4096
#endif
template <class EL, bool RELU, bool ROWS>
__global__ __launch_bounds__(256) void i8_colmax_vec_kernel(const bf16_t* x, int64_t ld, int64_t T, int64_t rows_per_block, int* emax,
                                                            const unsigned* rowmask, const RowsOut* rows_out) {
  __shared__ int best_lds[128];
  if (ROWS && rows_out->n_rows == 0) return;
  const int cg = threadIdx.x & 15, tl = threadIdx.x >> 4;
  const int j0 = blockIdx.x * 128 + cg * 8;
  const int64_t t0 = (int64_t)blockIdx.y * rows_per_block + tl;
  const int64_t t1 = min(T, (int64_t)(blockIdx.y + 1) * rows_per_block);
  if (threadIdx.x < 128) best_lds[threadIdx.x] = 1;
  __syncthreads();
  int best[8] = {1, 1, 1, 1, 1, 1, 1, 1};
  for (int64_t t = t0; t < t1; t += 16) {
    i32x4 v = *(const i32x4*)(x + t * ld + j0);
    if (row_left<ROWS>(rowmask, t)) v = (i32x4)0;
#pragma unroll
    for (int q = 0; q < 4; q++) {
      const unsigned w = relu_pair<EL, RELU>((unsigned)v[q]);
      best[2 * q] = max(best[2 * q], EL::ee_if_nonzero(w & 0xFFFF));
      best[2 * q + 1] = max(best[2 * q + 1], EL::ee_if_nonzero(w >> 16));
    }
  }
#pragma unroll
  for (int q = 0; q < 8; q++) atomicMax(&best_lds[cg * 8 + q], best[q]);
  __syncthreads();
  if (threadIdx.x < 128) atomicMax(emax + blockIdx.x * 128 + threadIdx.x, best_lds[threadIdx.x]);
}

constexpr int SPLIT_TILES = 8;
template <class EL, bool RELU, bool ROWS>
__global__ __launch_bounds__(256) void i8_split_vec_kernel(const bf16_t* x, int64_t ld, int64_t T, int n, int nk, const int* emax,
                                                           signed char* planes, unsigned long long* stats, unsigned char* zmask,
                                                           const unsigned* rowmask) {
  __shared__ __attribute__((aligned(16))) bf16_t tile[64 * 128];
  __shared__ int st_lds[NSTAT + 1][128];
  const int f0 = blockIdx.x * 128;
  const int f = threadIdx.x & 127, ks = threadIdx.x >> 7;
  const int E = emax[f0 + f];
  const int64_t groups = n / 32;
  const int G = (f0 + f) >> 5, r = f & 31;
  for (int i = threadIdx.x; i < (NSTAT + 1) * 128; i += 256) (&st_lds[0][0])[i] = 0;
  int q[NSTAT + 1] = {};
  auto load_tile = [&](int tile_index, i32x4 (&v)[4]) {
    const int64_t tok0 = (int64_t)tile_index * 2 * KS;
#pragma unroll
    for (int c4 = 0; c4 < 4; c4++) {
      const int c = threadIdx.x + 256 * c4;
      const int64_t t = tok0 + (c >> 4);
      v[c4] = (i32x4)0;
      if (t < T && !row_left<ROWS>(rowmask, t)) v[c4] = *(const i32x4*)(x + t * ld + f0 + (c & 15) * 8);
    }
  };
  const int tile0 = blockIdx.y * SPLIT_TILES, tiles = (nk + 1) / 2;
  for (int it = 0; it < SPLIT_TILES && tile0 + it < tiles; it++) {
    __syncthreads();
    {
      i32x4 v[4];
      load_tile(tile0 + it, v);
#pragma unroll
      for (int c4 = 0; c4 < 4; c4++) *(i32x4*)(tile + (threadIdx.x + 256 * c4) * 8) = v[c4];
    }
    __syncthreads();
    const int kt = (tile0 + it) * 2 + ks;
    if (kt >= nk) continue;
    unsigned any[NP] = {};
    unsigned deep_dig[2][NP - ALWAYS_WRITTEN_PLANES][4];
#pragma unroll
    for (int h = 0; h < 2; h++) {
      unsigned dig[NP][4];
#pragma unroll
      for (int q4 = 0; q4 < 4; q4++) {
        unsigned lo[4], hi[4];
#pragma unroll
        for (int e = 0; e < 4; e++) {
          int sig, ee;
          EL::parts(relu_bits<EL, RELU>(tile[(ks * 32 + h * 16 + q4 * 4 + e) * 128 + f]), sig, ee);
          q[NSTAT - 1] += (sig != 0);
          bool rounded;
          const long long N = fixed_point<EL>(sig, E - ee, rounded);
          if (rounded) q[NSTAT] += (sig != 0);
          const unsigned long long biased = (unsigned long long)N + 0x0000008080808080ull;
          lo[e] = (unsigned)biased;
          hi[e] = (unsigned)(biased >> 32);
        }
#pragma unroll
        for (int s2 = 0; s2 < NP; s2++) {
          constexpr unsigned ZERO_HI = 0x0c0c0000u;
          const int byte = NP - 1 - s2;
          const unsigned sel = ZERO_HI | (unsigned)(byte & 3) | ((4u + (unsigned)(byte & 3)) << 8);
          const unsigned t01 = __builtin_amdgcn_perm(byte < 4 ? lo[1] : hi[1], byte < 4 ? lo[0] : hi[0], sel);
          const unsigned t23 = __builtin_amdgcn_perm(byte < 4 ? lo[3] : hi[3], byte < 4 ? lo[2] : hi[2], sel);
          unsigned w = t01 | (t23 << 16);
          if (s2 > 0) w ^= 0x80808080u;
          dig[s2][q4] = w;
          q[s2] = __builtin_amdgcn_sdot4((int)w, (int)w, q[s2], false);
        }
        q[STAT_D0D1] = __builtin_amdgcn_sdot4((int)dig[0][q4], (int)dig[1][q4], q[STAT_D0D1], false);
      }
#pragma unroll
      for (int s2 = 0; s2 < NP; s2++) {
        any[s2] |= dig[s2][0] | dig[s2][1] | dig[s2][2] | dig[s2][3];
        if (s2 < ALWAYS_WRITTEN_PLANES) {
          signed char* piece = planes + ((s2 * groups + G) * (int64_t)nk + kt) * 1024;
          *(i32x4*)(piece + h * 512 + r * 16) = (i32x4){(int)dig[s2][0], (int)dig[s2][1], (int)dig[s2][2], (int)dig[s2][3]};
        } else {
#pragma unroll
          for (int i = 0; i < 4; i++) deep_dig[h][s2 - ALWAYS_WRITTEN_PLANES][i] = dig[s2][i];
        }
      }
    }
    const unsigned present = write_piece_mask(any, zmask, (int64_t)kt * groups + G);
#pragma unroll
    for (int s2 = ALWAYS_WRITTEN_PLANES; s2 < NP; s2++)
      if ((present >> s2) != 0) {
        signed char* piece = planes + ((s2 * groups + G) * (int64_t)nk + kt) * 1024;
#pragma unroll
        for (int h = 0; h < 2; h++)
          *(i32x4*)(piece + h * 512 + r * 16) = (i32x4){(int)deep_dig[h][s2 - ALWAYS_WRITTEN_PLANES][0], (int)deep_dig[h][s2 - ALWAYS_WRITTEN_PLANES][1],
                                                        (int)deep_dig[h][s2 - ALWAYS_WRITTEN_PLANES][2], (int)deep_dig[h][s2 - ALWAYS_WRITTEN_PLANES][3]};
      }
  }
  __syncthreads();
#pragma unroll
  for (int i = 0; i <= NSTAT; i++)
    if (q[i]) atomicAdd(&st_lds[i][f], q[i]);
  __syncthreads();
  if (threadIdx.x < 128) {
    unsigned long long* o = stats + f0 + threadIdx.x;
#pragma unroll
    for (int i = 0; i < STAT_COUNTS; i++) {
      const int val = st_lds[i][threadIdx.x];
      if (val) atomicAdd(o + (int64_t)i * n, (unsigned long long)(long long)val);
    }
    const unsigned long long counts = (unsigned long long)(unsigned)st_lds[NSTAT - 1][threadIdx.x] |
                                      ((unsigned long long)(unsigned)st_lds[NSTAT][threadIdx.x] << 32);
    if (counts) atomicAdd(o + (int64_t)STAT_COUNTS * n, counts);
  }
}

}

int enqueue_colmax(const I8Call& c, int i, bool masked) {
  const I8Stat& s = c.stat[i];
  const int n = s.n;
  I8Call k = c;
  k.rows = masked;
  const unsigned* mask = masked ? s.rowmask : nullptr;
  const RowsOut* ro = masked ? s.rows_out : nullptr;
  if (s.vec()) {
    const int64_t slabs = std::min(ceil_div(c.n_tokens, (int64_t)64), std::max((int64_t)1, (int64_t)MDG_COLMAX_WGS / (n / 128)));
    const int64_t rows_vec = ceil_div(ceil_div(c.n_tokens, slabs), (int64_t)16) * 16;
    MDG_I8_DISPATCH_ROWS(k, i8_colmax_vec_kernel, dim3((unsigned)(n / 128), (unsigned)ceil_div(c.n_tokens, rows_vec)), dim3(256), 0, c.st,
                         s.x, s.ld, c.n_tokens, rows_vec, s.emax, mask, ro);
  } else {
    const int64_t rows_per_block = 2048;
    MDG_I8_DISPATCH_ROWS(k, i8_colmax_kernel, dim3((unsigned)ceil_div(n, 64), (unsigned)ceil_div(c.n_tokens, rows_per_block)), dim3(256),
                         0, c.st, s.x, s.ld, c.n_tokens, n, rows_per_block, s.emax, mask, ro);
  }
  MDG_LAUNCH_CHECK();
  return MDG_OK;
}

int enqueue_split(const I8Call& c, int i) {
  const I8Stat& s = c.stat[i];
  const int n = s.n, nk = c.nk;
  MDG_HIP(hipMemsetAsync(s.emax, 0, ints_bytes(n), c.st));
  MDG_TRY(enqueue_colmax(c, i, false));
  if (c.rows) {
    MDG_TRY(enqueue_row_selection(c, i));
    MDG_TRY(enqueue_colmax(c, i, true));
  }
  if (s.vec()) {
    MDG_I8_DISPATCH_ROWS(c, i8_split_vec_kernel, dim3((unsigned)(n / 128), (unsigned)ceil_div(nk, 2 * SPLIT_TILES)), dim3(256), 0, c.st, s.x,
                         s.ld, c.n_tokens, n, nk, s.emax, s.planes, s.stats(), s.zmask, (const unsigned*)s.rowmask);
  } else {
    MDG_I8_DISPATCH_ROWS(c, i8_split_kernel, dim3((unsigned)(n / 32), (unsigned)ceil_div(nk, SPLIT_STEPS)), dim3(256), 0, c.st, s.x, s.ld,
                         c.n_tokens, n, nk, s.emax, s.planes, s.stats(), s.zmask, (const unsigned*)s.rowmask);
  }
  MDG_LAUNCH_CHECK();
  return MDG_OK;
}

}
```

Baseline: 1.178.

## Batch per-problem int8 covariance passes into single multi-problem launches

```diff
diff --git a/modegpt_amd/csrc/common.hpp b/modegpt_amd/csrc/common.hpp
--- a/modegpt_amd/csrc/common.hpp
+++ b/modegpt_amd/csrc/common.hpp
@@ -29,6 +29,8 @@
 int cov_accum_gated(const void* x, int dtype, int64_t n_tokens, int64_t n_feat, int64_t batch, int64_t ld, int relu, double* sigma,
                     int64_t ld_sigma, int64_t sigma_bs, void* ws, size_t ws_bytes, const int* gate, int gate_mask, int gate_want,
                     void* stream);
+int cov_accum_gated_multi(int count, const mdg_cov_problem* problems, int dtype, int relu, void* const* ws, const int* const* gate,
+                          int gate_mask, int gate_want, void* stream);
 #define MDG_CHECK_ARG(cond, ...)            \
   do {                                      \
     if (!(cond)) {                          \
diff --git a/modegpt_amd/csrc/cov.hip b/modegpt_amd/csrc/cov.hip
--- a/modegpt_amd/csrc/cov.hip
+++ b/modegpt_amd/csrc/cov.hip
@@ -263,6 +263,53 @@
   tri_decode(t, bi, bj);
   if (bi == bj) cov_tile<DT, false, true, true>(a, lds, b, bi, bj, split, slot);
   else cov_tile<DT, false, true, false>(a, lds, b, bi, bj, split, slot);
+}
+
+template <int DT, bool RELU, bool ALL_FAST>
+__global__ __launch_bounds__(256, 2) void cov_accum_gated_multi_kernel(CovMulti m) {
+  __shared__ double lds[4 * PANEL];
+  int u = blockIdx.x, pi = 0;
+  while (pi + 1 < m.n && u >= m.unit_start[pi + 1]) pi++;
+  u -= m.unit_start[pi];
+  const CovArgs& a = m.p[pi];
+  if (a.gate && (*a.gate & a.gate_mask) != a.gate_want) return;
+  const int tiles = a.batch * a.ntri;
+  const int split = u / tiles, slot = u % tiles;
+  const int b = slot / a.ntri, t = slot % a.ntri;
+  int bi, bj;
+  tri_decode(t, bi, bj);
+  if (ALL_FAST || a.vec_ok) {
+    if (bi == bj) cov_tile<DT, RELU, true, true>(a, lds, b, bi, bj, split, slot);
+    else cov_tile<DT, RELU, true, false>(a, lds, b, bi, bj, split, slot);
+  } else {
+    if (bi == bj) cov_tile<DT, RELU, false, true>(a, lds, b, bi, bj, split, slot);
+    else cov_tile<DT, RELU, false, false>(a, lds, b, bi, bj, split, slot);
+  }
+}
+
+struct CovReduceMulti {
+  CovMulti m;
+  int tile_start[MULTI_MAX + 1];
+};
+__global__ __launch_bounds__(256) void cov_reduce_multi_kernel(CovReduceMulti r) {
+  int u = blockIdx.x, pi = 0;
+  while (pi + 1 < r.m.n && u >= r.tile_start[pi + 1]) pi++;
+  u -= r.tile_start[pi];
+  const CovArgs& a = r.m.p[pi];
+  if (a.gate && (*a.gate & a.gate_mask) != a.gate_want) return;
+  const int b = u / a.ntri, t = u % a.ntri;
+  int bi, bj;
+  tri_decode(t, bi, bj);
+  double* sg = a.sigma + (int64_t)b * a.sigma_bs;
+  const int64_t tile_stride = (int64_t)(a.batch * a.ntri) * (TILE * TILE);
+  const double* pt = a.partial + (int64_t)u * (TILE * TILE);
+  const int e = blockIdx.y * 256 + threadIdx.x;
+  const int r_ = e / TILE, c = e % TILE;
+  const int64_t gr = (int64_t)bi * TILE + r_, gc = (int64_t)bj * TILE + c;
+  if (gr >= a.n_feat || gc >= a.n_feat) return;
+  double s = 0.;
+  for (int k = 0; k < a.ksplit; k++) s += pt[k * tile_stride + e];
+  sg[gr * a.ld_sigma + gc] += s;
 }
 
 __global__ __launch_bounds__(256) void cov_reduce_kernel(CovArgs a) {
@@ -467,6 +514,66 @@
   return MDG_OK;
 }
 
+template <int DT>
+static void launch_gated_multi(const CovMulti& m, int relu, bool all_fast, hipStream_t st) {
+  const dim3 grid((unsigned)m.unit_start[m.n]);
+  if (all_fast) {
+    if (relu) hipLaunchKernelGGL((cov_accum_gated_multi_kernel<DT, true, true>), grid, dim3(256), 0, st, m);
+    else hipLaunchKernelGGL((cov_accum_gated_multi_kernel<DT, false, true>), grid, dim3(256), 0, st, m);
+  } else {
+    if (relu) hipLaunchKernelGGL((cov_accum_gated_multi_kernel<DT, true, false>), grid, dim3(256), 0, st, m);
+    else hipLaunchKernelGGL((cov_accum_gated_multi_kernel<DT, false, false>), grid, dim3(256), 0, st, m);
+  }
+}
+
+int mdg::cov_accum_gated_multi(int count, const mdg_cov_problem* pr, int dtype, int relu, void* const* ws, const int* const* gate,
+                               int gate_mask, int gate_want, void* stream) {
+  MDG_CHECK_ARG(count >= 1 && count <= MULTI_MAX && pr && ws && gate, "cov_accum_gated_multi: 1..%d problems", MULTI_MAX);
+  MDG_CHECK_ARG(dtype == MDG_BF16 || dtype == MDG_F16, "cov_accum_gated_multi: bf16 or fp16 only (dtype %d)", dtype);
+  const size_t esz = dtype_size(dtype);
+  CovReduceMulti r;
+  CovMulti& m = r.m;
+  m.n = count;
+  int64_t units = 0, rtiles = 0;
+  bool all_fast = true;
+  for (int i = 0; i < count; i++) {
+    const mdg_cov_problem& q = pr[i];
+    MDG_CHECK_ARG(q.n_tokens > 0 && q.n_tokens == pr[0].n_tokens && q.n_feat > 0 && q.n_feat % TILE == 0 && q.batch > 0 && q.x && q.sigma &&
+                      q.ld >= q.n_feat * q.batch && q.ld_sigma >= q.n_feat,
+                  "cov_accum_gated_multi: problem %d: bad sizes", i);
+    CovArgs& a = m.p[i];
+    a.x = q.x; a.ld = q.ld; a.n_tokens = q.n_tokens; a.n_feat = (int)q.n_feat; a.batch = (int)q.batch;
+    a.tiles = (int)(q.n_feat / TILE); a.ntri = a.tiles * (a.tiles + 1) / 2;
+    a.sigma = q.sigma; a.ld_sigma = q.ld_sigma; a.sigma_bs = q.sigma_batch_stride;
+    a.ksplit = cov_ksplit(q.n_tokens, q.n_feat, q.batch, &a.tokens_per_split);
+    a.partial = (double*)ws[i];
+    a.gate = gate[i]; a.gate_mask = gate_mask; a.gate_want = gate_want;
+    a.vec_ok = ((uintptr_t)q.x % 16 == 0) && ((q.ld * esz) % 16 == 0);
+    all_fast = all_fast && a.vec_ok;
+    MDG_CHECK_ARG(a.ksplit == 1 || ws[i], "cov_accum_gated_multi: problem %d needs its split-K workspace", i);
+    const int64_t tiles = (int64_t)a.batch * a.ntri;
+    m.unit_start[i] = (int)units;
+    r.tile_start[i] = (int)rtiles;
+    units += tiles * a.ksplit;
+    if (a.ksplit > 1) rtiles += tiles;
+    MDG_CHECK_ARG(units < (1ll << 31), "cov_accum_gated_multi: grid too large");
+  }
+  for (int i = count; i <= MULTI_MAX; i++) {
+    m.unit_start[i] = (int)units;
+    r.tile_start[i] = (int)rtiles;
+    if (i < MULTI_MAX) m.p[i] = m.p[0];
+  }
+  hipStream_t st = (hipStream_t)stream;
+  if (dtype == MDG_BF16) launch_gated_multi<MDG_BF16>(m, relu, all_fast, st);
+  else launch_gated_multi<MDG_F16>(m, relu, all_fast, st);
+  MDG_LAUNCH_CHECK();
+  if (rtiles) {
+    hipLaunchKernelGGL(cov_reduce_multi_kernel, dim3((unsigned)rtiles, TILE * TILE / 256), dim3(256), 0, st, r);
+    MDG_LAUNCH_CHECK();
+  }
+  return MDG_OK;
+}
+
 static int multi_ksplit(int64_t n_tokens, int64_t* tokens_per_split) {
   int64_t ks = n_tokens / 4096;
   if (ks < 1) ks = 1;
diff --git a/modegpt_amd/csrc/cov_i8.hip b/modegpt_amd/csrc/cov_i8.hip
--- a/modegpt_amd/csrc/cov_i8.hip
+++ b/modegpt_amd/csrc/cov_i8.hip
@@ -5,27 +5,31 @@
 namespace mdg {
 namespace {
 
-size_t layout(int count, const mdg_cov_problem* pr, void* ws, I8Call* out, size_t* fallback_off) {
-  size_t off = SHARED_BYTES + PARTIAL_BYTES, fb = 0;
+size_t layout(int count, const mdg_cov_problem* pr, void* ws, I8Call* out) {
+  size_t off = 0;
   char* const base = (char*)ws;
-  if (out) {
-    out->count = count;
-    out->n_tokens = pr[0].n_tokens;
-    out->nk = (int)ceil_div(pr[0].n_tokens, KS);
-    out->shared = (SharedBlock*)base;
-    out->partial = (double*)(base + SHARED_BYTES);
-  }
-  for (int i = 0; i < count; i++) {
-    const int64_t cols = pr[i].n_feat * pr[i].batch, T = pr[i].n_tokens;
+  auto take = [&](size_t bytes) { char* p = base ? base + off : nullptr; off += bytes; return p; };
+  I8Stat st[MAX_PROBLEMS];
+  const int64_t T = pr[0].n_tokens;
+  SharedBlock* const shared = (SharedBlock*)take(SHARED_BYTES);
+  for (int i = 0; i < count; i++) st[i].emax = (int*)take(align_up(ints_bytes(pr[i].n_feat * pr[i].batch), 256));
+  const size_t zero_bytes = off;
+  double* const partial = (double*)take(PARTIAL_BYTES);
+  const RowsWsBytes rw = rows_ws_bytes(T);
+  for (int i = 0; i < count; i++) {
+    st[i].rowmask = (unsigned*)take(rw.mask);
+    st[i].votes = (int*)take(rw.votes);
+    st[i].rows_out = (RowsOut*)take(rw.out);
+  }
+  for (int i = 0; i < count; i++) {
+    const int64_t cols = pr[i].n_feat * pr[i].batch;
     const LoWsBytes lo = lo_ws_bytes(T, cols);
-    I8Stat s;
+    I8Stat& s = st[i];
     s.x = (const bf16_t*)pr[i].x; s.ld = pr[i].ld;
     s.sigma = pr[i].sigma; s.ld_sigma = pr[i].ld_sigma;
     s.n = (int)cols; s.block = pr[i].batch > 1 ? TI : 0;
-    s.route_flag = out ? out->shared->route_flag + i : nullptr;
-    auto take = [&](size_t bytes) { char* p = base ? base + off : nullptr; off += bytes; return p; };
+    s.route_flag = base ? shared->route_flag + i : nullptr;
     s.planes = (signed char*)take(align_up((size_t)NP * (size_t)cols * (size_t)ceil_div(T, KS) * KS, 256));
-    s.emax = (int*)take(align_up(ints_bytes(cols), 256));
     s.vals = (double*)take(align_up(route_vals_bytes(cols), 256));
     s.route = (RouteOut*)take(align_up(sizeof(RouteOut), 256));
     s.colpart = (double*)take(align_up(column_partials_bytes(cols), 256));
@@ -35,15 +39,35 @@
     s.lo_xd = (bf16_t*)take(align_up(lo.xd, 256));
     s.lo_rentries = (LoEntry*)take(lo.rentries);
     s.lo_rtotals = (int*)take(align_up(lo.rtotals, 256));
-    const RowsWsBytes rw = rows_ws_bytes(T);
-    s.rowmask = (unsigned*)take(rw.mask);
-    s.votes = (int*)take(rw.votes);
-    s.rows_out = (RowsOut*)take(rw.out);
-    if (out) out->stat[i] = s;
-    fb = std::max(fb, mdg_cov_accum_ws_bytes(T, pr[i].n_feat, pr[i].batch));
-  }
-  if (fallback_off) *fallback_off = off;
-  return off + fb + 256;
+  }
+  if (out) {
+    out->count = count;
+    out->n_tokens = T;
+    out->nk = (int)ceil_div(T, KS);
+    out->shared = shared;
+    out->partial = partial;
+    out->zero_bytes = zero_bytes;
+    out->rows_zero_bytes = (size_t)count * (rw.mask + rw.votes + rw.out);
+    out->pass = PassTable{};
+    out->pass.count = count;
+    out->pass.nk = out->nk;
+    out->pass.T = T;
+  }
+  for (int i = 0; i < count; i++) {
+    if (out) {
+      const I8Stat& s = st[i];
+      out->stat[i] = s;
+      out->fallback_off[i] = off;
+      PassStat& q = out->pass.s[i];
+      q.x = s.x; q.ld = s.ld; q.n = s.n; q.block = s.block; q.vec = s.vec();
+      q.emax = s.emax; q.stats = s.stats(); q.planes = s.planes; q.zmask = s.zmask;
+      q.rowmask = s.rowmask; q.votes = s.votes; q.rows_out = s.rows_out;
+      q.vals = s.vals; q.route = s.route; q.route_flag = s.route_flag; q.colpart = s.colpart;
+      q.sigma = s.sigma; q.ld_sigma = s.ld_sigma;
+    }
+    off += align_up(mdg_cov_accum_ws_bytes(T, pr[i].n_feat, pr[i].batch), 256);
+  }
+  return off + 256;
 }
 
 bool problems_ok(int count, const mdg_cov_problem* pr) {
@@ -65,7 +89,7 @@
 
 extern "C" size_t mdg_cov_accum_i8_multi_ws_bytes(int count, const mdg_cov_problem* problems) {
   if (!problems_ok(count, problems) || problems[0].n_tokens == 0) return 0;
-  return layout(count, problems, nullptr, nullptr, nullptr);
+  return layout(count, problems, nullptr, nullptr);
 }
 
 extern "C" int mdg_cov_accum_i8_multi(int count, const mdg_cov_problem* problems, void* ws, size_t ws_bytes, double tolerance, int flags,
@@ -88,30 +112,30 @@
   if (problems[0].n_tokens == 0) return MDG_OK;
   for (int i = 0; i < count; i++) MDG_CHECK_ARG(problems[i].x && problems[i].sigma, "mdg_cov_accum_i8_multi: null pointer");
   I8Call c;
-  size_t fb_off = 0;
-  const size_t need = layout(count, problems, ws, &c, &fb_off);
+  const size_t need = layout(count, problems, ws, &c);
   MDG_CHECK_ARG(ws && ws_bytes >= need, "mdg_cov_accum_i8_multi: workspace %zu < required %zu", ws_bytes, need);
   c.route_counts = route_counts;
   c.st = (hipStream_t)stream;
   c.f16 = (flags & MDG_I8_F16) != 0;
   c.relu = (flags & MDG_I8_RELU) != 0;
   c.rows = (flags & MDG_I8_ROWS) != 0;
-  MDG_HIP(hipMemsetAsync(c.shared, 0, SHARED_BYTES, c.st));
+  MDG_HIP(hipMemsetAsync(c.shared, 0, c.zero_bytes, c.st));
   if (c.rows) MDG_HIP(hipMemsetAsync(&c.shared->rows_flag, 1, 1, c.st));
-  for (int i = 0; i < count; i++) {
-    MDG_TRY(enqueue_split(c, i));
-    MDG_TRY(enqueue_route(c, i, tolerance));
-  }
+  MDG_TRY(enqueue_split(c));
+  MDG_TRY(enqueue_route(c, tolerance));
   if (offer_exact) MDG_TRY(enqueue_lo_lists(c, exact_always));
   MDG_TRY(enqueue_products(c, offer_exact, ev_start, ev_stop));
   if (offer_exact) MDG_TRY(enqueue_lo_products(c, exact_always));
-  for (int i = 0; i < count; i++) MDG_TRY(enqueue_columns(c, i));
-  if (c.rows)
-    for (int i = 0; i < count; i++) MDG_TRY(enqueue_rows_product(c, i));
-  for (int i = 0; i < count; i++) {
-    const mdg_cov_problem& q = problems[i];
-    MDG_TRY(cov_accum_gated(q.x, c.f16 ? MDG_F16 : MDG_BF16, c.n_tokens, q.n_feat, q.batch, q.ld, c.relu ? 1 : 0, q.sigma, q.ld_sigma, q.sigma_batch_stride, (char*)ws + fb_off,
-                            ws_bytes - fb_off, c.stat[i].route_flag, 2, 2, stream));
+  MDG_TRY(enqueue_columns(c));
+  if (c.rows) MDG_TRY(enqueue_rows_product(c));
+  {
+    void* fb_ws[MAX_PROBLEMS];
+    const int* gates[MAX_PROBLEMS];
+    for (int i = 0; i < count; i++) {
+      fb_ws[i] = (char*)ws + c.fallback_off[i];
+      gates[i] = c.stat[i].route_flag;
+    }
+    MDG_TRY(cov_accum_gated_multi(count, problems, c.f16 ? MDG_F16 : MDG_BF16, c.relu ? 1 : 0, fb_ws, gates, 2, 2, stream));
   }
   MDG_TRY(report_product_diagnostics(c));
   if (used_i8) {
@@ -160,7 +184,7 @@
   MDG_CLEAR();
   MDG_CHECK_ARG(problems_ok(count, problems) && stat >= 0 && stat < count && ws, "mdg_cov_accum_i8_route: bad arguments");
   I8Call c;
-  layout(count, problems, const_cast<void*>(ws), &c, nullptr);
+  layout(count, problems, const_cast<void*>(ws), &c);
   RouteOut r;
   SharedBlock shared;
   hipStream_t st = (hipStream_t)stream;
@@ -204,7 +228,7 @@
   MDG_CLEAR();
   MDG_CHECK_ARG(problems_ok(count, problems) && stat >= 0 && stat < count && ws, "mdg_cov_accum_i8_rows: bad arguments");
   I8Call c;
-  layout(count, problems, const_cast<void*>(ws), &c, nullptr);
+  layout(count, problems, const_cast<void*>(ws), &c);
   RowsOut r;
   MDG_TRY(read_rows(c, stat, &r, (hipStream_t)stream));
   if (n_rows) *n_rows = r.n_rows;
diff --git a/modegpt_amd/csrc/cov_i8.hpp b/modegpt_amd/csrc/cov_i8.hpp
--- a/modegpt_amd/csrc/cov_i8.hpp
+++ b/modegpt_amd/csrc/cov_i8.hpp
@@ -91,6 +91,30 @@
       if ((c).relu) hipLaunchKernelGGL((KERNEL<Bf16Elem, true, false>), __VA_ARGS__);     \
       else hipLaunchKernelGGL((KERNEL<Bf16Elem, false, false>), __VA_ARGS__);             \
     }                                                                                     \
+  } while (0)
+#define MDG_I8_DISPATCH_ROWS_K(c, K, KERNEL, ...)                                         \
+  do {                                                                                    \
+    if ((c).rows) {                                                                       \
+      if ((c).f16) {                                                                      \
+        if ((c).relu) hipLaunchKernelGGL((KERNEL<F16Elem, true, true, K>), __VA_ARGS__);  \
+        else hipLaunchKernelGGL((KERNEL<F16Elem, false, true, K>), __VA_ARGS__);          \
+      } else {                                                                            \
+        if ((c).relu) hipLaunchKernelGGL((KERNEL<Bf16Elem, true, true, K>), __VA_ARGS__); \
+        else hipLaunchKernelGGL((KERNEL<Bf16Elem, false, true, K>), __VA_ARGS__);         \
+      }                                                                                   \
+    } else if ((c).f16) {                                                                 \
+      if ((c).relu) hipLaunchKernelGGL((KERNEL<F16Elem, true, false, K>), __VA_ARGS__);   \
+      else hipLaunchKernelGGL((KERNEL<F16Elem, false, false, K>), __VA_ARGS__);           \
+    } else {                                                                              \
+      if ((c).relu) hipLaunchKernelGGL((KERNEL<Bf16Elem, true, false, K>), __VA_ARGS__);  \
+      else hipLaunchKernelGGL((KERNEL<Bf16Elem, false, false, K>), __VA_ARGS__);          \
+    }                                                                                     \
+  } while (0)
+#define MDG_I8_DISPATCH_KINDS(c, kinds, KERNEL, ...)                                      \
+  do {                                                                                    \
+    if ((kinds) == 1) MDG_I8_DISPATCH_ROWS_K(c, 1, KERNEL, __VA_ARGS__);                  \
+    else if ((kinds) == 2) MDG_I8_DISPATCH_ROWS_K(c, 2, KERNEL, __VA_ARGS__);             \
+    else MDG_I8_DISPATCH_ROWS_K(c, 3, KERNEL, __VA_ARGS__);                               \
   } while (0)
 template <bool ROWS>
 __device__ __forceinline__ bool row_left(const unsigned* rowmask, int64_t t) {
@@ -162,10 +186,60 @@
   bool vec() const { return (uintptr_t)x % 16 == 0 && ld % 8 == 0; }
   unsigned long long* stats() const { return (unsigned long long*)(emax + (n + 1) / 2 * 2); }
 };
+struct PassStat {
+  const bf16_t* x;
+  int64_t ld;
+  int n, block, vec;
+  int* emax;
+  unsigned long long* stats;
+  signed char* planes;
+  unsigned char* zmask;
+  unsigned* rowmask;
+  int* votes;
+  RowsOut* rows_out;
+  double* vals;
+  RouteOut* route;
+  int* route_flag;
+  double* colpart;
+  double* sigma;
+  int64_t ld_sigma;
+};
+struct PassTable {
+  int count, nk;
+  int64_t T;
+  PassStat s[MAX_PROBLEMS];
+};
+struct PassGrid {
+  int start[MAX_PROBLEMS + 1];
+  int gx[MAX_PROBLEMS];
+  int64_t aux[MAX_PROBLEMS];
+  int total() const { return start[MAX_PROBLEMS]; }
+};
+inline bool pass_grid_add(PassGrid& g, int i, int64_t gx, int64_t gy, int64_t aux = 0) {
+  const int64_t end = (int64_t)g.start[i] + gx * gy;
+  if (gx < 1 || gy < 1 || end >= (1ll << 31)) return false;
+  g.gx[i] = (int)gx;
+  g.aux[i] = aux;
+  for (int k = i + 1; k <= MAX_PROBLEMS; k++) g.start[k] = (int)end;
+  return true;
+}
+#ifdef __HIPCC__
+__device__ __forceinline__ int pass_stat_of(const PassGrid& g, int count, unsigned& w) {
+  int p = 0;
+  while (p + 1 < count && (int)w >= g.start[p + 1]) p++;
+  w -= (unsigned)g.start[p];
+  return p;
+}
+#endif
+
 struct I8Call {
   int count, nk;
   int64_t n_tokens;
   I8Stat stat[MAX_PROBLEMS];
+  PassTable pass;
+  size_t zero_bytes;
+  size_t rows_zero_bytes;
+  size_t fallback_off[MAX_PROBLEMS];
   bool f16, relu;
   bool rows;
   SharedBlock* shared;
@@ -177,16 +251,16 @@
 inline size_t ints_bytes(int64_t n) { return (size_t)((n + 1) / 2 * 2) * sizeof(int) + (size_t)(NSTAT * n) * sizeof(unsigned long long) + sizeof(RouteScratch); }
 
 #pragma GCC visibility push(hidden)
-int enqueue_split(const I8Call& c, int i);
-int enqueue_colmax(const I8Call& c, int i, bool masked);
+int enqueue_split(const I8Call& c);
+int enqueue_colmax(const I8Call& c, bool masked);
 struct RowsWsBytes { size_t mask, votes, out; };
 RowsWsBytes rows_ws_bytes(int64_t n_tokens);
-int enqueue_row_selection(const I8Call& c, int i);
-int enqueue_rows_product(const I8Call& c, int i);
+int enqueue_row_selection(const I8Call& c);
+int enqueue_rows_product(const I8Call& c);
 size_t route_vals_bytes(int64_t n);
 size_t column_partials_bytes(int64_t n);
-int enqueue_route(const I8Call& c, int i, double tolerance);
-int enqueue_columns(const I8Call& c, int i);
+int enqueue_route(const I8Call& c, double tolerance);
+int enqueue_columns(const I8Call& c);
 struct LoWsBytes { size_t entries, counts, xd, rentries, rtotals; };
 LoWsBytes lo_ws_bytes(int64_t n_tokens, int64_t n);
 int enqueue_lo_lists(const I8Call& c, bool always);
diff --git a/modegpt_amd/csrc/cov_i8_route.hip b/modegpt_amd/csrc/cov_i8_route.hip
--- a/modegpt_amd/csrc/cov_i8_route.hip
+++ b/modegpt_amd/csrc/cov_i8_route.hip
@@ -47,9 +47,20 @@
   unsigned min_nnz;
 };
 
-__global__ __launch_bounds__(ROUTE_THREADS) void i8_route_kernel(const unsigned long long* __restrict__ stats, int* emax, int n, int64_t n_tokens,
-                                                                 double* __restrict__ vals, RoutePartial* partial, RouteScratch* scratch,
-                                                                 int* flag, RouteOut* out, int* route_counts, double tolerance) {
+__global__ __launch_bounds__(ROUTE_THREADS) void i8_route_kernel(PassTable table, PassGrid grid, int* route_counts, double tolerance) {
+  unsigned bx = blockIdx.x;
+  const int pi = pass_stat_of(grid, table.count, bx);
+  const unsigned nwg = (unsigned)(grid.start[pi + 1] - grid.start[pi]);
+  const PassStat& ps = table.s[pi];
+  const unsigned long long* __restrict__ stats = ps.stats;
+  int* const emax = ps.emax;
+  const int n = ps.n;
+  const int64_t n_tokens = table.T;
+  double* __restrict__ vals = ps.vals;
+  RoutePartial* const partial = (RoutePartial*)(ps.vals + (size_t)NVAL * n);
+  RouteScratch* const scratch = (RouteScratch*)(ps.stats + (size_t)NSTAT * n);
+  int* const flag = ps.route_flag;
+  RouteOut* const out = ps.route;
   __shared__ unsigned long long group_max[NVAL][64];
   __shared__ Top2 wave_top[ROUTE_THREADS / 64][NVAL];
   __shared__ Top2 top[NVAL];
@@ -87,7 +98,7 @@
 #pragma unroll
   for (int i = 0; i < NVAL; i++) t[i] = Top2{-1.0, 0x7fffffff, -1.0};
   {
-    const int j = blockIdx.x * ROUTE_THREADS + tid;
+    const int j = bx * ROUTE_THREADS + tid;
     bool nonfinite = false;
     if (j < n) {
       double q[NSTAT];
@@ -119,7 +130,7 @@
     if (lane == 0 && nf) atomicAdd(&scratch->forced, __popcll(nf));
   }
   reduce_top(t);
-  RoutePartial& mine = partial[blockIdx.x];
+  RoutePartial& mine = partial[bx];
   if (tid < NVAL) mine.top[tid] = top[tid];
   if (tid == 0) mine.min_nnz = min_nnz;
   for (int i = tid; i < NVAL * 64; i += ROUTE_THREADS) (&mine.cls[0][0])[i] = (&group_max[0][0])[i];
@@ -127,9 +138,8 @@
   __syncthreads();
   if (tid == 0) my_ticket = atomicAdd(&scratch->ticket, 1);
   __syncthreads();
-  if (my_ticket != (int)gridDim.x - 1) return;
+  if (my_ticket != (int)nwg - 1) return;
   __threadfence();
-  const unsigned nwg = gridDim.x;
   if (tid < NVAL) {
     Top2 r = partial[0].top[tid];
     unsigned w = 1;
@@ -288,9 +298,14 @@
   for (int j = tid; j < n; j += ROUTE_THREADS) emax[j] &= 255;
 }
 
-__global__ __launch_bounds__(256) void i8_clear_columns_kernel(const RouteOut* route, const int* flag, const int* emax, signed char* planes,
-                                                               unsigned char* zmask, int n, int nk) {
-  if ((*flag & 2) || (int)blockIdx.x >= route->n_out) return;
+__global__ __launch_bounds__(256) void i8_clear_columns_kernel(PassTable table) {
+  const PassStat& ps = table.s[blockIdx.z];
+  const RouteOut* const route = ps.route;
+  if ((*ps.route_flag & 2) || (int)blockIdx.x >= route->n_out) return;
+  const int* const emax = ps.emax;
+  signed char* const planes = ps.planes;
+  unsigned char* const zmask = ps.zmask;
+  const int n = ps.n, nk = table.nk;
   const int j = route->out[blockIdx.x];
   const int64_t groups = n / 32;
   const int G = j >> 5, lane = threadIdx.x & 63, row = lane & 31;
@@ -324,8 +339,22 @@
   const unsigned* rowmask;
 };
 
+__device__ __forceinline__ ColArgs col_args(const PassTable& t, const PassStat& s) {
+  ColArgs a;
+  a.x = s.x; a.ld = s.ld; a.T = t.T; a.n = s.n;
+  a.vec = s.vec;
+  a.route = s.route;
+  a.flag = s.route_flag;
+  a.part = s.colpart;
+  a.rowmask = s.rowmask;
+  return a;
+}
+
 template <class EL, bool RELU, bool ROWS>
-__global__ __launch_bounds__(64) void i8_columns_kernel(ColArgs a) {
+__global__ __launch_bounds__(64) void i8_columns_kernel(PassTable table, PassGrid grid) {
+  unsigned bx = blockIdx.x;
+  const int pi = pass_stat_of(grid, table.count, bx);
+  const ColArgs a = col_args(table, table.s[pi]);
   const int pass = blockIdx.z;
   const int n_out = a.route->n_out;
   if ((*a.flag & 2) || pass * COLK_GROUP >= n_out) return;
@@ -334,7 +363,7 @@
   const int lane = threadIdx.x;
   const int my_k = lane % COLK_GROUP;
   const int my_col = my_k < nj ? a.route->out[pass * COLK_GROUP + my_k] : -1;
-  const int c0 = blockIdx.x * COLK_WG_COLS + lane * 8;
+  const int c0 = bx * COLK_WG_COLS + lane * 8;
   const bool active = c0 < a.n;
   const int64_t chunk_len = (a.T + COLK_CHUNKS - 1) / COLK_CHUNKS;
   const int64_t t0 = blockIdx.y * chunk_len, t1 = min(a.T, t0 + chunk_len);
@@ -402,10 +431,18 @@
     }
 }
 
-__global__ __launch_bounds__(256) void i8_columns_reduce_kernel(ColArgs a, const int* emax, double* sigma, int64_t ld_sigma, int block) {
+__global__ __launch_bounds__(256) void i8_columns_reduce_kernel(PassTable table, PassGrid grid) {
+  unsigned bx = blockIdx.x;
+  const int pi = pass_stat_of(grid, table.count, bx);
+  const PassStat& ps = table.s[pi];
+  const ColArgs a = col_args(table, ps);
+  const int* const emax = ps.emax;
+  double* const sigma = ps.sigma;
+  const int64_t ld_sigma = ps.ld_sigma;
+  const int block = ps.block;
   const int k = blockIdx.y;
   if ((*a.flag & 2) || k >= a.route->n_out) return;
-  const int c = blockIdx.x * 256 + threadIdx.x;
+  const int c = bx * 256 + threadIdx.x;
   if (c >= a.n) return;
   const int j = a.route->out[k];
   if (block && c / block != j / block) return;
@@ -421,31 +458,24 @@
 size_t route_vals_bytes(int64_t n) { return (size_t)(NVAL * n) * sizeof(double) + (size_t)ceil_div(n, (int64_t)ROUTE_THREADS) * sizeof(RoutePartial); }
 size_t column_partials_bytes(int64_t n) { return (size_t)ROUTE_JMAX * COLK_CHUNKS * (size_t)n * sizeof(double); }
 
-int enqueue_route(const I8Call& c, int i, double tolerance) {
-  const I8Stat& s = c.stat[i];
-  const int n = s.n;
-  RoutePartial* partial = (RoutePartial*)(s.vals + (size_t)NVAL * n);
-  RouteScratch* scratch = (RouteScratch*)(s.stats() + (size_t)NSTAT * n);
-  hipLaunchKernelGGL(i8_route_kernel, dim3((unsigned)ceil_div(n, ROUTE_THREADS)), dim3(ROUTE_THREADS), 0, c.st, s.stats(), s.emax, n,
-                     c.n_tokens, s.vals, partial, scratch, s.route_flag, s.route, c.route_counts, tolerance);
-  hipLaunchKernelGGL(i8_clear_columns_kernel, dim3(ROUTE_JMAX, (unsigned)std::min(64, (c.nk + 3) / 4)), dim3(256), 0, c.st,
-                     (const RouteOut*)s.route, (const int*)s.route_flag, (const int*)s.emax, s.planes, s.zmask, n, c.nk);
+int enqueue_route(const I8Call& c, double tolerance) {
+  PassGrid g = {};
+  for (int i = 0; i < c.count; i++)
+    MDG_CHECK_ARG(pass_grid_add(g, i, ceil_div(c.stat[i].n, ROUTE_THREADS), 1), "mdg_cov_accum_i8_multi: route: grid too large");
+  hipLaunchKernelGGL(i8_route_kernel, dim3((unsigned)g.total()), dim3(ROUTE_THREADS), 0, c.st, c.pass, g, c.route_counts, tolerance);
+  hipLaunchKernelGGL(i8_clear_columns_kernel, dim3(ROUTE_JMAX, (unsigned)std::min(64, (c.nk + 3) / 4), (unsigned)c.count), dim3(256), 0, c.st,
+                     c.pass);
   MDG_LAUNCH_CHECK();
   return MDG_OK;
 }
 
-int enqueue_columns(const I8Call& c, int i) {
-  const I8Stat& s = c.stat[i];
-  ColArgs a;
-  a.x = s.x; a.ld = s.ld; a.T = c.n_tokens; a.n = s.n;
-  a.vec = s.vec();
-  a.route = s.route;
-  a.flag = s.route_flag;
-  a.part = s.colpart;
-  a.rowmask = s.rowmask;
-  MDG_I8_DISPATCH_ROWS(c, i8_columns_kernel, dim3((unsigned)ceil_div(s.n, COLK_WG_COLS), COLK_CHUNKS, ROUTE_JMAX / COLK_GROUP), dim3(64), 0, c.st, a);
-  hipLaunchKernelGGL(i8_columns_reduce_kernel, dim3((unsigned)ceil_div(s.n, 256), ROUTE_JMAX), dim3(256), 0, c.st, a, (const int*)s.emax, s.sigma,
-                     s.ld_sigma, s.block);
+int enqueue_columns(const I8Call& c) {
+  PassGrid g = {}, gr = {};
+  for (int i = 0; i < c.count; i++)
+    MDG_CHECK_ARG(pass_grid_add(g, i, ceil_div(c.stat[i].n, COLK_WG_COLS), 1) && pass_grid_add(gr, i, ceil_div(c.stat[i].n, 256), 1),
+                  "mdg_cov_accum_i8_multi: column kernel: grid too large");
+  MDG_I8_DISPATCH_ROWS(c, i8_columns_kernel, dim3((unsigned)g.total(), COLK_CHUNKS, ROUTE_JMAX / COLK_GROUP), dim3(64), 0, c.st, c.pass, g);
+  hipLaunchKernelGGL(i8_columns_reduce_kernel, dim3((unsigned)gr.total(), ROUTE_JMAX), dim3(256), 0, c.st, c.pass, gr);
   MDG_LAUNCH_CHECK();
   return MDG_OK;
 }
diff --git a/modegpt_amd/csrc/cov_i8_rows.hip b/modegpt_amd/csrc/cov_i8_rows.hip
--- a/modegpt_amd/csrc/cov_i8_rows.hip
+++ b/modegpt_amd/csrc/cov_i8_rows.hip
@@ -13,10 +13,17 @@
 constexpr int SELECT_THREADS = 1024;
 
 template <class EL, bool RELU>
-__global__ __launch_bounds__(256) void i8_row_votes_kernel(const bf16_t* x, int64_t ld, int64_t T, int n, int vec, const int* emax,
-                                                           int* votes) {
+__global__ __launch_bounds__(256) void i8_row_votes_kernel(PassTable table, PassGrid grid) {
   __shared__ __attribute__((aligned(16))) int thr[VOTE_SPAN];
-  const int c_begin = blockIdx.y * VOTE_SPAN;
+  unsigned by = blockIdx.y;
+  const int pi = pass_stat_of(grid, table.count, by);
+  const PassStat& ps = table.s[pi];
+  const bf16_t* const x = ps.x;
+  const int64_t ld = ps.ld, T = table.T;
+  const int n = ps.n, vec = ps.vec;
+  const int* const emax = ps.emax;
+  int* const votes = ps.votes;
+  const int c_begin = by * VOTE_SPAN;
   const int span = min(VOTE_SPAN, n - c_begin);
   for (int i = threadIdx.x; i < span; i += 256) thr[i] = max((emax[c_begin + i] & 255) - ROW_WINDOW, 1);
   __syncthreads();
@@ -55,9 +62,15 @@
   }
 }
 
-__global__ __launch_bounds__(SELECT_THREADS) void i8_row_select_kernel(const int* votes, int64_t T, int n, unsigned* rowmask, RowsOut* out,
-                                                                       int* emax) {
+__global__ __launch_bounds__(SELECT_THREADS) void i8_row_select_kernel(PassTable table) {
   __shared__ int cnt[SELECT_THREADS];
+  const PassStat& ps = table.s[blockIdx.x];
+  const int* const votes = ps.votes;
+  const int64_t T = table.T;
+  const int n = ps.n;
+  unsigned* const rowmask = ps.rowmask;
+  RowsOut* const out = ps.rows_out;
+  int* const emax = ps.emax;
   const int tid = threadIdx.x;
   const int64_t chunk = (T + SELECT_THREADS - 1) / SELECT_THREADS;
   const int64_t a = min(T, tid * chunk), b = min(T, a + chunk);
@@ -101,18 +114,27 @@
 };
 
 template <class EL, bool RELU>
-__global__ __launch_bounds__(256) void i8_rows_product_kernel(RowArgs a) {
+__global__ __launch_bounds__(256) void i8_rows_product_kernel(PassTable table, PassGrid grid, int* route_counts) {
   __shared__ __attribute__((aligned(16))) double lds[2 * PANEL];
   __shared__ int tok[ROWS_MAX];
+  unsigned bx = blockIdx.x;
+  const int pi = pass_stat_of(grid, table.count, bx);
+  const PassStat& ps = table.s[pi];
+  RowArgs a;
+  a.x = ps.x; a.ld = ps.ld; a.block = ps.block;
+  a.rows = ps.rows_out;
+  a.flag = ps.route_flag;
+  a.sigma = ps.sigma; a.ld_sigma = ps.ld_sigma;
+  a.route_counts = route_counts;
   const int nr = a.rows->n_rows;
   if (nr == 0 || (*a.flag & 2)) return;
   int bi, bj;
-  if (a.block) bi = bj = blockIdx.x;
-  else tri_decode(blockIdx.x, bi, bj);
+  if (a.block) bi = bj = bx;
+  else tri_decode(bx, bi, bj);
   const int tid = threadIdx.x, lane = tid & 63, wave = tid >> 6;
   const int wr = wave >> 1, wc = wave & 1;
   if (tid < ROWS_MAX) tok[tid] = tid < nr ? a.rows->rows[tid] : -1;
-  if (blockIdx.x == 0 && tid == 0 && a.route_counts) atomicAdd(a.route_counts + 5, nr);
+  if (bx == 0 && tid == 0 && a.route_counts) atomicAdd(a.route_counts + 5, nr);
   __syncthreads();
   const bool diag = bi == bj;
   double* const As = lds;
@@ -161,28 +183,25 @@
   return b;
 }
 
-int enqueue_row_selection(const I8Call& c, int i) {
-  const I8Stat& s = c.stat[i];
-  const RowsWsBytes b = rows_ws_bytes(c.n_tokens);
-  MDG_HIP(hipMemsetAsync(s.rowmask, 0, b.mask + b.votes + b.out, c.st));
-  MDG_I8_DISPATCH(c, i8_row_votes_kernel, dim3((unsigned)ceil_div(c.n_tokens, (int64_t)VOTE_TOKENS), (unsigned)ceil_div(s.n, VOTE_SPAN)),
-                  dim3(256), 0, c.st, s.x, s.ld, c.n_tokens, s.n, (int)s.vec(), (const int*)s.emax, s.votes);
-  hipLaunchKernelGGL(i8_row_select_kernel, dim3(1), dim3(SELECT_THREADS), 0, c.st, (const int*)s.votes, c.n_tokens, s.n, s.rowmask,
-                     s.rows_out, s.emax);
+int enqueue_row_selection(const I8Call& c) {
+  MDG_HIP(hipMemsetAsync(c.stat[0].rowmask, 0, c.rows_zero_bytes, c.st));
+  PassGrid g = {};
+  for (int i = 0; i < c.count; i++)
+    MDG_CHECK_ARG(pass_grid_add(g, i, 1, ceil_div(c.stat[i].n, VOTE_SPAN)), "mdg_cov_accum_i8_multi: vote pass: grid too large");
+  MDG_I8_DISPATCH(c, i8_row_votes_kernel, dim3((unsigned)ceil_div(c.n_tokens, (int64_t)VOTE_TOKENS), (unsigned)g.total()), dim3(256), 0, c.st,
+                  c.pass, g);
+  hipLaunchKernelGGL(i8_row_select_kernel, dim3((unsigned)c.count), dim3(SELECT_THREADS), 0, c.st, c.pass);
   MDG_LAUNCH_CHECK();
   return MDG_OK;
 }
 
-int enqueue_rows_product(const I8Call& c, int i) {
-  const I8Stat& s = c.stat[i];
-  RowArgs a;
-  a.x = s.x; a.ld = s.ld; a.block = s.block;
-  a.rows = s.rows_out;
-  a.flag = s.route_flag;
-  a.sigma = s.sigma; a.ld_sigma = s.ld_sigma;
-  a.route_counts = c.route_counts;
-  const int64_t nb = s.n / TILE;
-  MDG_I8_DISPATCH(c, i8_rows_product_kernel, dim3((unsigned)(s.block ? nb : nb * (nb + 1) / 2)), dim3(256), 0, c.st, a);
+int enqueue_rows_product(const I8Call& c) {
+  PassGrid g = {};
+  for (int i = 0; i < c.count; i++) {
+    const int64_t nb = c.stat[i].n / TILE;
+    MDG_CHECK_ARG(pass_grid_add(g, i, c.stat[i].block ? nb : nb * (nb + 1) / 2, 1), "mdg_cov_accum_i8_multi: row kernel: grid too large");
+  }
+  MDG_I8_DISPATCH(c, i8_rows_product_kernel, dim3((unsigned)g.total()), dim3(256), 0, c.st, c.pass, g, c.route_counts);
   MDG_LAUNCH_CHECK();
   return MDG_OK;
 }
diff --git a/modegpt_amd/csrc/cov_i8_split.hip b/modegpt_amd/csrc/cov_i8_split.hip
--- a/modegpt_amd/csrc/cov_i8_split.hip
+++ b/modegpt_amd/csrc/cov_i8_split.hip
@@ -15,12 +15,12 @@
 }
 
 template <class EL, bool RELU, bool ROWS>
-__global__ __launch_bounds__(256) void i8_colmax_kernel(const bf16_t* x, int64_t ld, int64_t T, int n, int64_t rows_per_block,
-                                                        int* emax, const unsigned* rowmask, const RowsOut* rows_out) {
+__device__ __forceinline__ void colmax_body(const bf16_t* x, int64_t ld, int64_t T, int n, int64_t rows_per_block, int* emax,
+                                            const unsigned* rowmask, const RowsOut* rows_out, unsigned bx, unsigned by) {
   if (ROWS && rows_out->n_rows == 0) return;
-  const int j = blockIdx.x * 64 + (threadIdx.x & 63);
-  const int64_t t0 = (int64_t)blockIdx.y * rows_per_block + (threadIdx.x >> 6);
-  const int64_t t1 = min(T, (int64_t)(blockIdx.y + 1) * rows_per_block);
+  const int j = bx * 64 + (threadIdx.x & 63);
+  const int64_t t0 = (int64_t)by * rows_per_block + (threadIdx.x >> 6);
+  const int64_t t1 = min(T, (int64_t)(by + 1) * rows_per_block);
   int best = 1;
   if (j < n)
     for (int64_t t = t0; t < t1; t += 4) {
@@ -45,12 +45,12 @@
 
 constexpr int SPLIT_STEPS = 64;
 template <class EL, bool RELU, bool ROWS>
-__global__ __launch_bounds__(256) void i8_split_kernel(const bf16_t* x, int64_t ld, int64_t T, int n, int nk, const int* emax,
-                                                       signed char* planes, unsigned long long* stats, unsigned char* zmask,
-                                                       const unsigned* rowmask) {
+__device__ __forceinline__ void split_body(const bf16_t* x, int64_t ld, int64_t T, int n, int nk, const int* emax, signed char* planes,
+                                           unsigned long long* stats, unsigned char* zmask, const unsigned* rowmask, unsigned bx,
+                                           unsigned by) {
   __shared__ unsigned long long st_lds[NSTAT][32];
   const int r = threadIdx.x & 31;
-  const int G = blockIdx.x;
+  const int G = bx;
   const int j = G * 32 + r;
   const int E = emax[j];
   const int64_t groups = n / 32;
@@ -58,7 +58,7 @@
   __syncthreads();
   long long q[NSTAT] = {};
   for (int kq = 0; kq < SPLIT_STEPS; kq += 8) {
-    const int kt = blockIdx.y * SPLIT_STEPS + kq + (threadIdx.x >> 5);
+    const int kt = by * SPLIT_STEPS + kq + (threadIdx.x >> 5);
     if (kt >= nk) break;
     unsigned any[NP] = {};
 #pragma unroll
@@ -106,14 +106,14 @@
 #define MDG_COLMAX_WGS 4096
 #endif
 template <class EL, bool RELU, bool ROWS>
-__global__ __launch_bounds__(256) void i8_colmax_vec_kernel(const bf16_t* x, int64_t ld, int64_t T, int64_t rows_per_block, int* emax,
-                                                            const unsigned* rowmask, const RowsOut* rows_out) {
+__device__ __forceinline__ void colmax_vec_body(const bf16_t* x, int64_t ld, int64_t T, int64_t rows_per_block, int* emax,
+                                                const unsigned* rowmask, const RowsOut* rows_out, unsigned bx, unsigned by) {
   __shared__ int best_lds[128];
   if (ROWS && rows_out->n_rows == 0) return;
   const int cg = threadIdx.x & 15, tl = threadIdx.x >> 4;
-  const int j0 = blockIdx.x * 128 + cg * 8;
-  const int64_t t0 = (int64_t)blockIdx.y * rows_per_block + tl;
-  const int64_t t1 = min(T, (int64_t)(blockIdx.y + 1) * rows_per_block);
+  const int j0 = bx * 128 + cg * 8;
+  const int64_t t0 = (int64_t)by * rows_per_block + tl;
+  const int64_t t1 = min(T, (int64_t)(by + 1) * rows_per_block);
   if (threadIdx.x < 128) best_lds[threadIdx.x] = 1;
   __syncthreads();
   int best[8] = {1, 1, 1, 1, 1, 1, 1, 1};
@@ -130,17 +130,17 @@
 #pragma unroll
   for (int q = 0; q < 8; q++) atomicMax(&best_lds[cg * 8 + q], best[q]);
   __syncthreads();
-  if (threadIdx.x < 128) atomicMax(emax + blockIdx.x * 128 + threadIdx.x, best_lds[threadIdx.x]);
+  if (threadIdx.x < 128) atomicMax(emax + bx * 128 + threadIdx.x, best_lds[threadIdx.x]);
 }
 
 constexpr int SPLIT_TILES = 8;
 template <class EL, bool RELU, bool ROWS>
-__global__ __launch_bounds__(256) void i8_split_vec_kernel(const bf16_t* x, int64_t ld, int64_t T, int n, int nk, const int* emax,
-                                                           signed char* planes, unsigned long long* stats, unsigned char* zmask,
-                                                           const unsigned* rowmask) {
+__device__ __forceinline__ void split_vec_body(const bf16_t* x, int64_t ld, int64_t T, int n, int nk, const int* emax, signed char* planes,
+                                               unsigned long long* stats, unsigned char* zmask, const unsigned* rowmask, unsigned bx,
+                                               unsigned by) {
   __shared__ __attribute__((aligned(16))) bf16_t tile[64 * 128];
   __shared__ int st_lds[NSTAT + 1][128];
-  const int f0 = blockIdx.x * 128;
+  const int f0 = bx * 128;
   const int f = threadIdx.x & 127, ks = threadIdx.x >> 7;
   const int E = emax[f0 + f];
   const int64_t groups = n / 32;
@@ -157,7 +157,7 @@
       if (t < T && !row_left<ROWS>(rowmask, t)) v[c4] = *(const i32x4*)(x + t * ld + f0 + (c & 15) * 8);
     }
   };
-  const int tile0 = blockIdx.y * SPLIT_TILES, tiles = (nk + 1) / 2;
+  const int tile0 = by * SPLIT_TILES, tiles = (nk + 1) / 2;
   for (int it = 0; it < SPLIT_TILES && tile0 + it < tiles; it++) {
     __syncthreads();
     {
@@ -244,45 +244,71 @@
   }
 }
 
-}
-
-int enqueue_colmax(const I8Call& c, int i, bool masked) {
-  const I8Stat& s = c.stat[i];
-  const int n = s.n;
+template <class EL, bool RELU, bool ROWS, int KINDS>
+__global__ __launch_bounds__(256) void i8_colmax_kernel(PassTable t, PassGrid g) {
+  unsigned w = blockIdx.x;
+  const int pi = pass_stat_of(g, t.count, w);
+  const PassStat& s = t.s[pi];
+  const unsigned bx = w % (unsigned)g.gx[pi], by = w / (unsigned)g.gx[pi];
+  if (KINDS == 1 || (KINDS == 3 && s.vec)) colmax_vec_body<EL, RELU, ROWS>(s.x, s.ld, t.T, g.aux[pi], s.emax, s.rowmask, s.rows_out, bx, by);
+  else colmax_body<EL, RELU, ROWS>(s.x, s.ld, t.T, s.n, g.aux[pi], s.emax, s.rowmask, s.rows_out, bx, by);
+}
+
+template <class EL, bool RELU, bool ROWS, int KINDS>
+__global__ __launch_bounds__(256) void i8_split_kernel(PassTable t, PassGrid g) {
+  unsigned w = blockIdx.x;
+  const int pi = pass_stat_of(g, t.count, w);
+  const PassStat& s = t.s[pi];
+  const unsigned bx = w % (unsigned)g.gx[pi], by = w / (unsigned)g.gx[pi];
+  if (KINDS == 1 || (KINDS == 3 && s.vec)) split_vec_body<EL, RELU, ROWS>(s.x, s.ld, t.T, s.n, t.nk, s.emax, s.planes, s.stats, s.zmask, s.rowmask, bx, by);
+  else split_body<EL, RELU, ROWS>(s.x, s.ld, t.T, s.n, t.nk, s.emax, s.planes, s.stats, s.zmask, s.rowmask, bx, by);
+}
+
+int kinds_of(const I8Call& c) {
+  int kinds = 0;
+  for (int i = 0; i < c.count; i++) kinds |= c.stat[i].vec() ? 1 : 2;
+  return kinds;
+}
+
+}
+
+int enqueue_colmax(const I8Call& c, bool masked) {
   I8Call k = c;
   k.rows = masked;
-  const unsigned* mask = masked ? s.rowmask : nullptr;
-  const RowsOut* ro = masked ? s.rows_out : nullptr;
-  if (s.vec()) {
-    const int64_t slabs = std::min(ceil_div(c.n_tokens, (int64_t)64), std::max((int64_t)1, (int64_t)MDG_COLMAX_WGS / (n / 128)));
-    const int64_t rows_vec = ceil_div(ceil_div(c.n_tokens, slabs), (int64_t)16) * 16;
-    MDG_I8_DISPATCH_ROWS(k, i8_colmax_vec_kernel, dim3((unsigned)(n / 128), (unsigned)ceil_div(c.n_tokens, rows_vec)), dim3(256), 0, c.st,
-                         s.x, s.ld, c.n_tokens, rows_vec, s.emax, mask, ro);
-  } else {
-    const int64_t rows_per_block = 2048;
-    MDG_I8_DISPATCH_ROWS(k, i8_colmax_kernel, dim3((unsigned)ceil_div(n, 64), (unsigned)ceil_div(c.n_tokens, rows_per_block)), dim3(256),
-                         0, c.st, s.x, s.ld, c.n_tokens, n, rows_per_block, s.emax, mask, ro);
-  }
+  PassGrid g = {};
+  for (int i = 0; i < c.count; i++) {
+    const I8Stat& s = c.stat[i];
+    const int n = s.n;
+    bool ok;
+    if (s.vec()) {
+      const int64_t slabs = std::min(ceil_div(c.n_tokens, (int64_t)64), std::max((int64_t)1, (int64_t)MDG_COLMAX_WGS / (n / 128)));
+      const int64_t rows_vec = ceil_div(ceil_div(c.n_tokens, slabs), (int64_t)16) * 16;
+      ok = pass_grid_add(g, i, n / 128, ceil_div(c.n_tokens, rows_vec), rows_vec);
+    } else {
+      const int64_t rows_per_block = 2048;
+      ok = pass_grid_add(g, i, ceil_div(n, 64), ceil_div(c.n_tokens, rows_per_block), rows_per_block);
+    }
+    MDG_CHECK_ARG(ok, "mdg_cov_accum_i8_multi: maximum pass: grid too large");
+  }
+  MDG_I8_DISPATCH_KINDS(k, kinds_of(c), i8_colmax_kernel, dim3((unsigned)g.total()), dim3(256), 0, c.st, c.pass, g);
   MDG_LAUNCH_CHECK();
   return MDG_OK;
 }
 
-int enqueue_split(const I8Call& c, int i) {
-  const I8Stat& s = c.stat[i];
-  const int n = s.n, nk = c.nk;
-  MDG_HIP(hipMemsetAsync(s.emax, 0, ints_bytes(n), c.st));
-  MDG_TRY(enqueue_colmax(c, i, false));
+int enqueue_split(const I8Call& c) {
+  const int nk = c.nk;
+  MDG_TRY(enqueue_colmax(c, false));
   if (c.rows) {
-    MDG_TRY(enqueue_row_selection(c, i));
-    MDG_TRY(enqueue_colmax(c, i, true));
-  }
-  if (s.vec()) {
-    MDG_I8_DISPATCH_ROWS(c, i8_split_vec_kernel, dim3((unsigned)(n / 128), (unsigned)ceil_div(nk, 2 * SPLIT_TILES)), dim3(256), 0, c.st, s.x,
-                         s.ld, c.n_tokens, n, nk, s.emax, s.planes, s.stats(), s.zmask, (const unsigned*)s.rowmask);
-  } else {
-    MDG_I8_DISPATCH_ROWS(c, i8_split_kernel, dim3((unsigned)(n / 32), (unsigned)ceil_div(nk, SPLIT_STEPS)), dim3(256), 0, c.st, s.x, s.ld,
-                         c.n_tokens, n, nk, s.emax, s.planes, s.stats(), s.zmask, (const unsigned*)s.rowmask);
-  }
+    MDG_TRY(enqueue_row_selection(c));
+    MDG_TRY(enqueue_colmax(c, true));
+  }
+  PassGrid g = {};
+  for (int i = 0; i < c.count; i++) {
+    const I8Stat& s = c.stat[i];
+    const bool ok = s.vec() ? pass_grid_add(g, i, s.n / 128, ceil_div(nk, 2 * SPLIT_TILES)) : pass_grid_add(g, i, s.n / 32, ceil_div(nk, SPLIT_STEPS));
+    MDG_CHECK_ARG(ok, "mdg_cov_accum_i8_multi: split pass: grid too large");
+  }
+  MDG_I8_DISPATCH_KINDS(c, kinds_of(c), i8_split_kernel, dim3((unsigned)g.total()), dim3(256), 0, c.st, c.pass, g);
   MDG_LAUNCH_CHECK();
   return MDG_OK;
 }
```

After: 1.188 (median of 6 runs). Within noise of the previous version (+0.9%).
